# reczoo/RecBox

Hardware: AMD Instinct MI355X
Metric: samples/sec fwd+bwd, Criteo-shaped batch 65 536; embedding HBM GB/s vs roofline (higher is better)
Workload: dtype f32; 1 GPU; FM (recbox.ranking) Criteo-shaped 26 sparse + 13 dense, dim 16, batch 65536 per GPU, uniform ids (8 distinct batches resident in HBM, replayed in rotation), fused path, hipGraph replay (one captured step per resident batch), dense-grad autograd contract (persistent grad buffer, rows of the previous step re-zeroed), no optimiser step; global_batch=65536, batch_per_gpu=65536, parallelism=dp1

## Files before the change

include/recbox_hip.h:

```cpp
#ifndef RECBOX_HIP_H
#define RECBOX_HIP_H

#include <stddef.h>
#include <stdint.h>

#ifdef __cplusplus
extern "C" {
#endif

#define RBX_VERSION 124
#define RBX_MAX_FIELDS 64
#define RBX_NO_ID INT64_MIN

typedef enum {
  RBX_OK = 0,
  RBX_ERR_INVALID = -1,
  RBX_ERR_LAUNCH = -2,
  RBX_ERR_WORKSPACE = -3,
  RBX_ERR_UNSUPPORTED = -4
} rbx_status_t;

typedef enum { RBX_I32 = 0, RBX_I64 = 1, RBX_F32 = 2, RBX_F64 = 3 } rbx_dtype_t;

typedef enum {
  RBX_FIELD_CATEGORICAL = 0,
  RBX_FIELD_NUMERIC = 1,
  RBX_FIELD_DENSE = 2
} rbx_field_kind_t;

typedef enum {
  RBX_POOL_NONE = 0,
  RBX_POOL_SUM = 1,
  RBX_POOL_MEAN_VALUE = 2,
  RBX_POOL_MEAN_ID = 3,
  RBX_POOL_SUM_ID = 4,
  RBX_POOL_CONCAT = 5,
  RBX_POOL_MAX = 6
} rbx_pool_t;

typedef struct rbx_field {
  const void*  ids;
  const float* table;
  float*       grad;
  int64_t      ids_stride_b;
  int64_t      ids_stride_l;
  int64_t      vocab;
  int64_t      padding_idx;
  int64_t      mask_id;
  int64_t      out_off;
  int32_t      dim;
  int32_t      seq_len;
  int32_t      ids_dtype;
  int32_t      kind;
  int32_t      pool;
  float        eps;
  int64_t      table_stride;
} rbx_field_t;

const char* rbx_last_error(void);
int rbx_version(void);

int rbx_embed_fwd(const rbx_field_t* fields, int32_t n_fields, int64_t batch,
                  float* d_out, int64_t out_stride_b, float* d_row_scale,
                  int32_t* d_status, void* stream);

size_t rbx_embed_bwd_workspace_size(const rbx_field_t* fields, int32_t n_fields, int64_t batch);
int rbx_embed_sort(const rbx_field_t* fields, int32_t n_fields, int64_t batch,
                   void* d_workspace, size_t workspace_bytes, int32_t* d_status, void* stream);
int rbx_embed_bwd(const rbx_field_t* fields, int32_t n_fields, int64_t batch,
                  const float* d_dout, int64_t out_stride_b, const float* d_row_scale,
                  int32_t accumulate, void* d_workspace, size_t workspace_bytes, void* stream);
int rbx_embed_bwd_indexed(const rbx_field_t* fields, int32_t n_fields, int64_t batch,
                          const float* d_dout, int64_t out_stride_b, const int32_t* d_dout_index,
                          const float* d_row_scale, int32_t accumulate, void* d_workspace, size_t workspace_bytes,
                          void* stream);

#define RBX_MAX_BAGS 32
typedef struct rbx_bag {
  const void*  indices;
  const void*  offsets;
  const float* table;
  float*       grad;
  int64_t      nnz;
  int64_t      indices_stride;
  int64_t      vocab;
  int64_t      padding_idx;
  int64_t      mask_id;
  int64_t      out_off;
  int32_t      dim;
  int32_t      indices_dtype;
  int32_t      offsets_dtype;
  int32_t      pool;
  float        eps;
  int32_t      reserved;
} rbx_bag_t;
int rbx_embed_csr_fwd(const rbx_bag_t* bags, int32_t n_bags, int64_t batch, float* d_out, int64_t out_stride_b,
                      float* d_row_scale, int32_t* d_status, void* stream);
size_t rbx_embed_csr_bwd_workspace_size(const rbx_bag_t* bags, int32_t n_bags, int64_t batch);
int rbx_embed_csr_sort(const rbx_bag_t* bags, int32_t n_bags, int64_t batch, void* d_workspace, size_t workspace_bytes,
                       int32_t* d_status, void* stream);
int rbx_embed_csr_bwd(const rbx_bag_t* bags, int32_t n_bags, int64_t batch, const float* d_dout, int64_t out_stride_b,
                      const float* d_row_scale, int32_t accumulate, void* d_workspace, size_t workspace_bytes,
                      void* stream);
int rbx_embed_csr_fwd_weighted(const rbx_bag_t* bags, int32_t n_bags, int64_t batch, const float* const* d_weights,
                               float* d_out, int64_t out_stride_b, int32_t* d_status, void* stream);
int rbx_embed_csr_sort_weighted(const rbx_bag_t* bags, int32_t n_bags, int64_t batch, void* d_workspace,
                                size_t workspace_bytes, int32_t* d_status, void* stream);
int rbx_embed_csr_bwd_weighted(const rbx_bag_t* bags, int32_t n_bags, int64_t batch, const float* const* d_weights,
                               const float* d_dout, int64_t out_stride_b, int32_t accumulate, void* d_workspace,
                               size_t workspace_bytes, void* stream);
int rbx_embed_csr_weight_grad(const rbx_bag_t* bags, int32_t n_bags, int64_t batch, const float* d_dout,
                              int64_t out_stride_b, float* const* d_dweights, int32_t* d_status, void* stream);
int rbx_embed_csr_rezero(const rbx_bag_t* bags, int32_t n_bags, int64_t batch, void* d_workspace, size_t workspace_bytes,
                         void* stream);
struct rbx_opt;
int rbx_embed_csr_sparse_update(const rbx_bag_t* bags, int32_t n_bags, int64_t batch, const void* d_workspace,
                                size_t workspace_bytes, const struct rbx_opt* opt, float* const* d_state1,
                                float* const* d_state2, int32_t clear_grad, void* stream);
size_t rbx_embed_csr_fwd_max_workspace_size(const rbx_bag_t* bags, int32_t n_bags, int64_t batch, int64_t long_threshold);
int rbx_embed_csr_fwd_max(const rbx_bag_t* bags, int32_t n_bags, int64_t batch, int64_t long_threshold, float* d_out,
                          int64_t out_stride_b, int32_t* d_argpos, int64_t arg_stride_b, void* d_workspace,
                          size_t workspace_bytes, int32_t* d_status, void* stream);
int rbx_embed_csr_bwd_max(const rbx_bag_t* bags, int32_t n_bags, int64_t batch, const float* d_dout, int64_t out_stride_b,
                          const int32_t* d_argpos, int64_t arg_stride_b, int32_t accumulate, void* d_workspace,
                          size_t workspace_bytes, void* stream);

#define RBX_CSR_SEGMENT 256
#define RBX_CSR_WS_SEGMENTS 0
#define RBX_CSR_WS_LONG_BAGS 1
size_t rbx_embed_csr_fwd_long_workspace_size(const rbx_bag_t* bags, int32_t n_bags, int64_t batch, int64_t long_threshold);
int rbx_embed_csr_fwd_long(const rbx_bag_t* bags, int32_t n_bags, int64_t batch, int64_t long_threshold, float* d_out,
                           int64_t out_stride_b, float* d_row_scale, void* d_workspace, size_t workspace_bytes,
                           int32_t* d_status, void* stream);
int rbx_embed_csr_fwd_weighted_long(const rbx_bag_t* bags, int32_t n_bags, int64_t batch, int64_t long_threshold,
                                    const float* const* d_weights, float* d_out, int64_t out_stride_b, void* d_workspace,
                                    size_t workspace_bytes, int32_t* d_status, void* stream);
int rbx_embed_csr_weight_grad_long(const rbx_bag_t* bags, int32_t n_bags, int64_t batch, int64_t long_threshold,
                                   const float* d_dout, int64_t out_stride_b, float* const* d_dweights, void* d_workspace,
                                   size_t workspace_bytes, int32_t* d_status, void* stream);

int rbx_interaction_fwd(const float* d_emb, int64_t emb_stride_b, int64_t batch, int32_t n_fields, int32_t dim,
                        int32_t mode, float* d_out, void* stream);
int rbx_interaction_bwd(const float* d_emb, int64_t emb_stride_b, const float* d_dout, int64_t batch, int32_t n_fields,
                        int32_t dim, int32_t mode, float* d_demb, int64_t demb_stride_b, void* stream);

int rbx_pairmul_fwd(const float* d_left, const float* d_right, int64_t batch, int32_t n_fields, int32_t dim,
                    int32_t per_pair, float* d_out, void* stream);
int rbx_pairmul_bwd(const float* d_left, const float* d_right, const float* d_dout, int64_t batch, int32_t n_fields,
                    int32_t dim, int32_t per_pair, float* d_dleft, float* d_dright, void* stream);

int rbx_fm_fwd(const rbx_field_t* emb, const rbx_field_t* lr, int32_t n_fields, int64_t batch,
               const float* d_lr_bias, const float* d_extra, int32_t n_extra, int32_t extra_stride,
               int32_t extra_lr_off, const int32_t* d_extra_index, int64_t extra_rows, float* d_logit,
               float* d_prob, float* d_sum, int32_t* d_status, void* stream);
int rbx_fm_extra_bwd(const float* d_dlogit, const float* d_sum, const float* d_extra, int64_t batch,
                     int32_t n_extra, int32_t dim, int32_t extra_stride, int32_t extra_lr_off,
                     const int32_t* d_extra_index, int64_t extra_rows, float* d_dextra, void* stream);

size_t rbx_route_workspace_size(int64_t n_lookups, int32_t world);
int rbx_route(const rbx_field_t* tables, int32_t n_tables, int64_t batch, int32_t world, int64_t capacity,
              const int64_t* d_base, int64_t* d_send, int32_t* d_slot, uint8_t* d_overflow, void* d_workspace,
              size_t workspace_bytes, void* stream);
int rbx_route32(const rbx_field_t* tables, int32_t n_tables, int64_t batch, int32_t world, int64_t capacity,
                const int64_t* d_base, int32_t* d_send, int32_t* d_slot, uint8_t* d_overflow, void* d_workspace,
                size_t workspace_bytes, void* stream);

typedef struct rbx_shard_geom {
  int32_t world;
  int32_t dim;
  int32_t n_rows;
  int32_t n_pool;
  int64_t batch;
  int64_t cap_rows;
  int64_t cap_pool;
} rbx_shard_geom_t;
size_t rbx_shard_int_chunk(const rbx_shard_geom_t* geom);
size_t rbx_shard_float_rows(const rbx_shard_geom_t* geom);
size_t rbx_shard_route_workspace_size(const rbx_shard_geom_t* geom, int32_t pool_seq_len);
int rbx_shard_route(const rbx_shard_geom_t* geom, const rbx_field_t* row_fields, const rbx_field_t* pool_field,
                    const int64_t* d_base, int32_t* d_send, int32_t* d_slot, float* d_inv, uint8_t* d_overflow,
                    int32_t* d_status, void* d_workspace, size_t workspace_bytes, void* stream);
int rbx_shard_serve(const rbx_shard_geom_t* geom, const int32_t* d_recv, const float* d_weight, int64_t n_local_rows,
                    float* d_back, int32_t* d_keys, int32_t* d_src, int32_t* d_status, void* stream);
int rbx_shard_combine_fwd(const rbx_shard_geom_t* geom, const float* d_back, const int32_t* d_slot, const float* d_inv,
                          float* d_out, int64_t out_stride_b, const int64_t* col_off, void* stream);
int rbx_shard_combine_bwd(const rbx_shard_geom_t* geom, const float* d_dout, int64_t dout_stride_b,
                          const int64_t* col_off, const int32_t* d_slot, const float* d_inv, float* d_gsend,
                          void* stream);
size_t rbx_fm_bwd_workspace_size(const rbx_field_t* emb, const rbx_field_t* lr, int32_t n_fields, int64_t batch);
int rbx_fm_sort(const rbx_field_t* emb, const rbx_field_t* lr, int32_t n_fields, int64_t batch,
                void* d_workspace, size_t workspace_bytes, int32_t* d_status, void* stream);
int rbx_fm_sort_phases(const rbx_field_t* emb, const rbx_field_t* lr, int32_t n_fields, int64_t batch,
                       void* d_workspace, size_t workspace_bytes, int32_t* d_status, int32_t phases, void* stream);
int rbx_fm_bwd(const rbx_field_t* emb, const rbx_field_t* lr, int32_t n_fields, int64_t batch,
               const float* d_dlogit, const float* d_sum, float* d_dbias, int32_t accumulate,
               int32_t phases, void* d_workspace, size_t workspace_bytes, void* stream);
int rbx_fm_quad(int32_t enable);
int rbx_sort_chained(int32_t enable);
int rbx_fm_rezero(const rbx_field_t* emb, const rbx_field_t* lr, int32_t n_fields, int64_t batch,
                  void* d_workspace, size_t workspace_bytes, void* stream);
int rbx_fm_head(const rbx_field_t* emb, const rbx_field_t* lr, int32_t n_fields, int64_t batch,
                const void* d_rezero_workspace, size_t rezero_workspace_bytes, void* d_sort_workspace,
                size_t sort_workspace_bytes, int32_t* d_status, void* stream);
int rbx_sort_share(const rbx_field_t* src_a, const rbx_field_t* src_b, int32_t src_n, int32_t src_is_fm,
                   const void* d_src_workspace, const rbx_field_t* dst_a, const rbx_field_t* dst_b, int32_t dst_n,
                   int32_t dst_is_fm, void* d_dst_workspace, size_t dst_workspace_bytes, int64_t batch, void* stream);
int rbx_embed_rezero(const rbx_field_t* fields, int32_t n_fields, int64_t batch, void* d_workspace,
                     size_t workspace_bytes, void* stream);

typedef enum { RBX_OPT_SGD = 0, RBX_OPT_ADAGRAD = 1, RBX_OPT_ADAM = 2 } rbx_opt_kind_t;
typedef struct rbx_opt {
  int32_t kind;
  float   lr;
  float   beta1, beta2;
  float   eps;
  float   weight_decay;
  const float* d_step_size;
} rbx_opt_t;
int rbx_opt_advance(int32_t kind, float lr, float beta1, float beta2, float lr_decay, float* d_t, float* d_step_size,
// ... 327 lines not shown
```

recbox_amd/_lib.py:

```python
import ctypes
import os

HERE = os.path.dirname(os.path.abspath(__file__))
LIB_PATH = os.environ.get("RECBOX_HIP_LIB") or os.path.join(HERE, "lib", "librecbox_hip.so")

RBX_MAX_FIELDS = 64
RBX_NO_ID = -(1 << 63)

RBX_OK, RBX_ERR_INVALID, RBX_ERR_LAUNCH, RBX_ERR_WORKSPACE, RBX_ERR_UNSUPPORTED = 0, -1, -2, -3, -4
RBX_I32, RBX_I64, RBX_F32, RBX_F64 = 0, 1, 2, 3
RBX_MASK_U8 = 4
FIELD_CATEGORICAL, FIELD_NUMERIC, FIELD_DENSE = 0, 1, 2
POOL_NONE, POOL_SUM, POOL_MEAN_VALUE, POOL_MEAN_ID, POOL_SUM_ID, POOL_CONCAT, POOL_MAX = 0, 1, 2, 3, 4, 5, 6
INTERACTION_MODES = {"product_sum": 0, "bi_interaction": 1, "inner_product": 2, "elementwise_product": 3}
FM_SORT_IDS, FM_SORT_TIER_B, FM_SORT_TIER_A = 1, 2, 4
FM_BWD_TABLES, FM_BWD_NUMERIC, FM_BWD_STORE, FM_BWD_SKIP_TIER_A, FM_BWD_SKIP_TIER_B = 1, 2, 4, 8, 16


class rbx_field_t(ctypes.Structure):
    _fields_ = [("ids", ctypes.c_void_p),
                ("table", ctypes.c_void_p),
                ("grad", ctypes.c_void_p),
                ("ids_stride_b", ctypes.c_int64),
                ("ids_stride_l", ctypes.c_int64),
                ("vocab", ctypes.c_int64),
                ("padding_idx", ctypes.c_int64),
                ("mask_id", ctypes.c_int64),
                ("out_off", ctypes.c_int64),
                ("dim", ctypes.c_int32),
                ("seq_len", ctypes.c_int32),
                ("ids_dtype", ctypes.c_int32),
                ("kind", ctypes.c_int32),
                ("pool", ctypes.c_int32),
                ("eps", ctypes.c_float),
                ("table_stride", ctypes.c_int64)]


RBX_MAX_BAGS = 32
STATUS_BAD_ID, STATUS_BAD_OFFSETS = 1, 2
CSR_SEGMENT = 256
CSR_WS_SEGMENTS, CSR_WS_LONG_BAGS = 0, 1


class rbx_bag_t(ctypes.Structure):
    _fields_ = [("indices", ctypes.c_void_p),
                ("offsets", ctypes.c_void_p),
                ("table", ctypes.c_void_p),
                ("grad", ctypes.c_void_p),
                ("nnz", ctypes.c_int64),
                ("indices_stride", ctypes.c_int64),
                ("vocab", ctypes.c_int64),
                ("padding_idx", ctypes.c_int64),
                ("mask_id", ctypes.c_int64),
                ("out_off", ctypes.c_int64),
                ("dim", ctypes.c_int32),
                ("indices_dtype", ctypes.c_int32),
                ("offsets_dtype", ctypes.c_int32),
                ("pool", ctypes.c_int32),
                ("eps", ctypes.c_float),
                ("reserved", ctypes.c_int32)]


class rbx_shard_geom_t(ctypes.Structure):
    _fields_ = [("world", ctypes.c_int32), ("dim", ctypes.c_int32), ("n_rows", ctypes.c_int32),
                ("n_pool", ctypes.c_int32), ("batch", ctypes.c_int64), ("cap_rows", ctypes.c_int64),
                ("cap_pool", ctypes.c_int64)]


class rbx_opt_t(ctypes.Structure):
    _fields_ = [("kind", ctypes.c_int32), ("lr", ctypes.c_float), ("beta1", ctypes.c_float), ("beta2", ctypes.c_float),
                ("eps", ctypes.c_float), ("weight_decay", ctypes.c_float), ("d_step_size", ctypes.c_void_p)]


OPT_SGD, OPT_ADAGRAD, OPT_ADAM = 0, 1, 2


class rbx_rowcopy_t(ctypes.Structure):
    _fields_ = [("src", ctypes.c_void_p), ("dst", ctypes.c_void_p), ("row_bytes", ctypes.c_int64)]


_P = ctypes.c_void_p
_FP = ctypes.POINTER(rbx_field_t)
_BP = ctypes.POINTER(rbx_bag_t)
_RP = ctypes.POINTER(rbx_rowcopy_t)
_GP = ctypes.POINTER(rbx_shard_geom_t)
_OP = ctypes.POINTER(rbx_opt_t)
_PP = ctypes.POINTER(ctypes.c_void_p)
_u64 = ctypes.c_uint64
_i32, _i64, _sz, _f32 = ctypes.c_int32, ctypes.c_int64, ctypes.c_size_t, ctypes.c_float
_IP = ctypes.POINTER(ctypes.c_int32)
_LP = ctypes.POINTER(ctypes.c_int64)

SIGNATURES = {
    "rbx_last_error": (ctypes.c_char_p, []),
    "rbx_version": (ctypes.c_int, []),
    "rbx_embed_fwd": (ctypes.c_int, [_FP, _i32, _i64, _P, _i64, _P, _P, _P]),
    "rbx_embed_bwd_workspace_size": (_sz, [_FP, _i32, _i64]),
    "rbx_embed_sort": (ctypes.c_int, [_FP, _i32, _i64, _P, _sz, _P, _P]),
    "rbx_embed_bwd": (ctypes.c_int, [_FP, _i32, _i64, _P, _i64, _P, _i32, _P, _sz, _P]),
    "rbx_embed_bwd_indexed": (ctypes.c_int, [_FP, _i32, _i64, _P, _i64, _P, _P, _i32, _P, _sz, _P]),
    "rbx_embed_csr_fwd": (ctypes.c_int, [_BP, _i32, _i64, _P, _i64, _P, _P, _P]),
    "rbx_embed_csr_bwd_workspace_size": (_sz, [_BP, _i32, _i64]),
    "rbx_embed_csr_sort": (ctypes.c_int, [_BP, _i32, _i64, _P, _sz, _P, _P]),
    "rbx_embed_csr_bwd": (ctypes.c_int, [_BP, _i32, _i64, _P, _i64, _P, _i32, _P, _sz, _P]),
    "rbx_embed_csr_fwd_weighted": (ctypes.c_int, [_BP, _i32, _i64, _PP, _P, _i64, _P, _P]),
    "rbx_embed_csr_sort_weighted": (ctypes.c_int, [_BP, _i32, _i64, _P, _sz, _P, _P]),
    "rbx_embed_csr_bwd_weighted": (ctypes.c_int, [_BP, _i32, _i64, _PP, _P, _i64, _i32, _P, _sz, _P]),
    "rbx_embed_csr_weight_grad": (ctypes.c_int, [_BP, _i32, _i64, _P, _i64, _PP, _P, _P]),
    "rbx_embed_csr_rezero": (ctypes.c_int, [_BP, _i32, _i64, _P, _sz, _P]),
    "rbx_embed_csr_sparse_update": (ctypes.c_int, [_BP, _i32, _i64, _P, _sz, _OP, _PP, _PP, _i32, _P]),
    "rbx_embed_csr_fwd_long_workspace_size": (_sz, [_BP, _i32, _i64, _i64]),
    "rbx_embed_csr_fwd_long": (ctypes.c_int, [_BP, _i32, _i64, _i64, _P, _i64, _P, _P, _sz, _P, _P]),
    "rbx_embed_csr_fwd_weighted_long": (ctypes.c_int, [_BP, _i32, _i64, _i64, _PP, _P, _i64, _P, _sz, _P, _P]),
    "rbx_embed_csr_weight_grad_long": (ctypes.c_int, [_BP, _i32, _i64, _i64, _P, _i64, _PP, _P, _sz, _P, _P]),
    "rbx_embed_csr_fwd_max_workspace_size": (_sz, [_BP, _i32, _i64, _i64]),
    "rbx_embed_csr_fwd_max": (ctypes.c_int, [_BP, _i32, _i64, _i64, _P, _i64, _P, _i64, _P, _sz, _P, _P]),
    "rbx_embed_csr_bwd_max": (ctypes.c_int, [_BP, _i32, _i64, _P, _i64, _P, _i64, _i32, _P, _sz, _P]),
    "rbx_shard_int_chunk": (_sz, [_GP]),
    "rbx_shard_float_rows": (_sz, [_GP]),
    "rbx_shard_route_workspace_size": (_sz, [_GP, _i32]),
    "rbx_shard_route": (ctypes.c_int, [_GP, _FP, _FP, _P, _P, _P, _P, _P, _P, _P, _sz, _P]),
    "rbx_shard_serve": (ctypes.c_int, [_GP, _P, _P, _i64, _P, _P, _P, _P, _P]),
    "rbx_shard_combine_fwd": (ctypes.c_int, [_GP, _P, _P, _P, _P, _i64, ctypes.POINTER(ctypes.c_int64), _P]),
    "rbx_shard_combine_bwd": (ctypes.c_int, [_GP, _P, _i64, ctypes.POINTER(ctypes.c_int64), _P, _P, _P, _P]),
    "rbx_interaction_fwd": (ctypes.c_int, [_P, _i64, _i64, _i32, _i32, _i32, _P, _P]),
    "rbx_interaction_bwd": (ctypes.c_int, [_P, _i64, _P, _i64, _i32, _i32, _i32, _P, _i64, _P]),
    "rbx_fm_fwd": (ctypes.c_int, [_FP, _FP, _i32, _i64, _P, _P, _i32, _i32, _i32, _P, _i64, _P, _P, _P, _P, _P]),
    "rbx_fm_extra_bwd": (ctypes.c_int, [_P, _P, _P, _i64, _i32, _i32, _i32, _i32, _P, _i64, _P, _P]),
    "rbx_route_workspace_size": (_sz, [_i64, _i32]),
    "rbx_route": (ctypes.c_int, [_FP, _i32, _i64, _i32, _i64, _P, _P, _P, _P, _P, _sz, _P]),
    "rbx_route32": (ctypes.c_int, [_FP, _i32, _i64, _i32, _i64, _P, _P, _P, _P, _P, _sz, _P]),
    "rbx_fm_bwd_workspace_size": (_sz, [_FP, _FP, _i32, _i64]),
    "rbx_fm_sort": (ctypes.c_int, [_FP, _FP, _i32, _i64, _P, _sz, _P, _P]),
    "rbx_fm_sort_phases": (ctypes.c_int, [_FP, _FP, _i32, _i64, _P, _sz, _P, _i32, _P]),
    "rbx_embed_sparse_update": (ctypes.c_int, [_FP, _i32, _i64, _P, _sz, _OP, _PP, _PP, _P]),
    "rbx_opt_advance": (ctypes.c_int, [_i32, _f32, _f32, _f32, _f32, _P, _P, _P]),
    "rbx_fm_sparse_update": (ctypes.c_int, [_FP, _FP, _i32, _i64, _P, _sz, _OP, _PP, _PP, _PP, _PP, _P]),
    "rbx_comm_bind": (ctypes.c_int, [_P, _P, _P, _P, _P]),
    "rbx_all_to_all": (ctypes.c_int, [_P, _P, _P, _sz, _i32, _P]),
    "rbx_comm_bind_collectives": (ctypes.c_int, [_P, _P, _P]),
    "rbx_all_reduce": (ctypes.c_int, [_P, _P, _P, _sz, _i32, _i32, _P]),
    "rbx_all_gather": (ctypes.c_int, [_P, _P, _P, _sz, _P]),
    "rbx_embed_rezero": (ctypes.c_int, [_FP, _i32, _i64, _P, _sz, _P]),
    "rbx_sort_share": (ctypes.c_int, [_FP, _FP, _i32, _i32, _P, _FP, _FP, _i32, _i32, _P, _sz, _i64, _P]),
    "rbx_rowscale": (ctypes.c_int, [_P, _P, _P, _i64, _i32, _f32, _P, _P]),
    "rbx_rowscale_seq": (ctypes.c_int, [_P, _P, _i64, _P, _i64, _i32, _f32, _P, _P]),
    "rbx_seq_colsum_workspace_size": (_sz, [_i64, _i32, _i32]),
    "rbx_seq_colsum": (ctypes.c_int, [_P, _P, _i64, _i32, _i32, _P, _P, _sz, _P]),
    "rbx_sum_prefix": (ctypes.c_int, [_P, _i64, _P, _i64, _P, _i64, _i64, _i32, _i32, _P, _i64, _P]),
    "rbx_fm_quad": (ctypes.c_int, [_i32]),
    "rbx_sort_chained": (ctypes.c_int, [_i32]),
    "rbx_fm_rezero": (ctypes.c_int, [_FP, _FP, _i32, _i64, _P, _sz, _P]),
    "rbx_fm_head": (ctypes.c_int, [_FP, _FP, _i32, _i64, _P, _sz, _P, _sz, _P, _P]),
    "rbx_fm_bwd": (ctypes.c_int, [_FP, _FP, _i32, _i64, _P, _P, _P, _i32, _i32, _P, _sz, _P]),
    "rbx_gatherdot_fwd": (ctypes.c_int, [_FP, _i32, _i64, _P, _i64, _f32, _P, _P, _P]),
    "rbx_gatherdot_bwd_workspace_size": (_sz, [_FP, _i32, _i64]),
    "rbx_gatherdot_sort": (ctypes.c_int, [_FP, _i32, _i64, _P, _sz, _P, _P]),
    "rbx_gatherdot_bwd": (ctypes.c_int, [_FP, _i32, _i64, _P, _i64, _P, _f32, _P, _i64, _i32, _P, _sz, _P]),
    "rbx_negsample": (ctypes.c_int, [_i64, _i64, _i32, _u64, _u64, _P, _P, _P, _P, _P, _P]),
    "rbx_negsample_checked": (ctypes.c_int, [_i64, _i64, _i32, _u64, _u64, _P, _P, _P, _P, _i64, _P, _P, _P]),
    "rbx_gather_rows": (ctypes.c_int, [_RP, _i32, _P, _i64, _i64, _P, _P]),
    "rbx_topk_workspace_size": (_sz, [_i64, _i64, _i32]),
    "rbx_topk": (ctypes.c_int, [_P, _P, _i64, _i64, _i64, _i32, _P, _P, _P, _sz, _P]),
    "rbx_penalize_members": (ctypes.c_int, [_P, _i64, _i32, _P, _P, _P, ctypes.c_double, _P, _P]),
    "rbx_membership": (ctypes.c_int, [_P, _i64, _i32, _P, _P, _P, _P, _P]),
    "rbx_search_ip_workspace_size": (_sz, [_i64, _i64, _i32, _i32]),
    "rbx_search_ip": (ctypes.c_int, [_P, _i64, _i64, _P, _i64, _i32, _i32, _P, _P, _P, _P, _sz, _P]),
    "rbx_batchnorm_workspace_size": (_sz, [_i64, _i32]),
    "rbx_batchnorm_fwd": (ctypes.c_int, [_P, _i64, _i32, _P, _P, _f32, _i32, _f32, _P, _P, _i32, _P, _P, _P, _P, _sz, _P]),
    "rbx_batchnorm_bwd": (ctypes.c_int, [_P, _P, _P, _i64, _i32, _P, _P, _P, _i32, _P, _P, _P, _P, _sz, _P]),
    "rbx_batchnorm_prelu_fwd": (ctypes.c_int, [_P, _i64, _i32, _P, _P, _P, _i32, _f32, _i32, _f32, _P, _P, _P, _P, _P, _P, _sz, _P]),
    "rbx_batchnorm_prelu_bwd": (ctypes.c_int, [_P, _P, _i64, _i32, _P, _P, _P, _i32, _P, _P, _i32, _P, _P, _P, _P, _P, _sz, _P]),
    "rbx_batchnorm_stats": (ctypes.c_int, [_P, _i64, _i32, _P, _P, _sz, _P]),
    "rbx_batchnorm_apply": (ctypes.c_int, [_P, _i64, _i32, _P, _P, _P, _P, _i32, _P, _P]),
    "rbx_batchnorm_bwd_reduce": (ctypes.c_int, [_P, _P, _P, _i64, _i32, _P, _P, _P, _P, _P, _sz, _P]),
    "rbx_batchnorm_bwd_dx": (ctypes.c_int, [_P, _P, _P, _i64, _i32, _P, _P, _P, _P, _P, _i64, _P, _P]),
    "rbx_cin_outer_fwd": (ctypes.c_int, [_P, _P, _i64, _i32, _i32, _i32, _P, _P]),
    "rbx_cin_outer_bwd": (ctypes.c_int, [_P, _P, _P, _i64, _i32, _i32, _i32, _P, _P, _P]),
    "rbx_act_workspace_size": (_sz, [_i64, _i32]),
    "rbx_prelu_fwd": (ctypes.c_int, [_P, _i64, _i32, _P, _i32, _P, _P]),
    "rbx_prelu_bwd": (ctypes.c_int, [_P, _P, _i64, _i32, _P, _i32, _P, _P, _P, _sz, _P]),
    "rbx_dropout": (ctypes.c_int, [_P, _i64, _f32, _u64, _P, _P, _P]),
    "rbx_dice_fwd": (ctypes.c_int, [_P, _i64, _i32, _P, _f32, _i32, _f32, _P, _P, _P, _P, _P, _P, _sz, _P]),
    "rbx_dice_bwd": (ctypes.c_int, [_P, _P, _i64, _i32, _P, _P, _P, _i32, _P, _P, _P, _sz, _P]),
    "rbx_layernorm_fwd": (ctypes.c_int, [_P, _i64, _i32, _P, _P, _f32, _P, _P, _P, _P]),
    "rbx_layernorm_bwd_workspace_size": (_sz, [_i64, _i32]),
    "rbx_layernorm_bwd": (ctypes.c_int, [_P, _P, _i64, _i32, _P, _P, _P, _P, _P, _P, _P, _sz, _P]),
    "rbx_cross_fwd": (ctypes.c_int, [_P, _P, _P, _P, _i64, _i32, _i32, _P, _P]),
    "rbx_cross_bwd": (ctypes.c_int, [_P, _P, _P, _i64, _i32, _i32, _P, _P, _P]),
    "rbx_bce_workspace_size": (_sz, [_i64]),
    "rbx_bce_mean_fwd": (ctypes.c_int, [_P, _P, _i64, _P, _P, _sz, _P]),
    "rbx_bce_mean_bwd": (ctypes.c_int, [_P, _P, _P, _i64, _P, _P]),
    "rbx_sigmoid_bce_mean": (ctypes.c_int, [_P, _P, _i64, _f32, _P, _P, _P, _P, _sz, _P]),
    "rbx_scale_by_scalar": (ctypes.c_int, [_P, _P, _i64, _P, _P]),
    "rbx_sigmoid_bce_mean_onepass": (ctypes.c_int, [_P, _P, _i64, _f32, _P, _P, _P, _P, _sz, _P, _P]),
    "rbx_pairmul_fwd": (ctypes.c_int, [_P, _P, _i64, _i32, _i32, _i32, _P, _P]),
    "rbx_pairmul_bwd": (ctypes.c_int, [_P, _P, _P, _i64, _i32, _i32, _i32, _P, _P, _P]),
    "rbx_l2norm_fwd": (ctypes.c_int, [_P, _i64, _i32, _f32, _P, _P, _P]),
    "rbx_l2norm_fwd_strided": (ctypes.c_int, [_P, _i64, _i64, _i64, _i32, _f32, _P, _P, _P]),
    "rbx_cosdot_fwd": (ctypes.c_int, [_P, _P, _i64, _i64, _i32, _i32, _f32, _f32, _P, _P, _P]),
    "rbx_cosdot_bwd": (ctypes.c_int, [_P, _P, _i64, _P, _P, _i64, _i32, _i32, _f32, _P, _P, _i64, _P]),
    "rbx_l2norm_bwd": (ctypes.c_int, [_P, _P, _P, _i64, _i32, _P, _P]),
    "rbx_pairdot_fwd": (ctypes.c_int, [_P, _P, _i64, _i32, _i32, _f32, _P, _P]),
    "rbx_pairdot_bwd": (ctypes.c_int, [_P, _P, _P, _i64, _i32, _i32, _f32, _P, _P, _P]),
    "rbx_linear_fwd": (ctypes.c_int, [_P, _i64, _P, _P, _i64, _i32, _i32, _i32, _P, _P]),
    "rbx_linear_bwd_workspace_size": (_sz, [_i64, _i32, _i32, _i32]),
    "rbx_linear_fwd_fused": (ctypes.c_int, [_P, _i64, _P, _P, _i64, _i32, _i32, _i32, _P, _i64, _P, _P, _i64, _P]),
    "rbx_linear_dx_fused": (ctypes.c_int, [_P, _i64, _P, _i64, _i32, _i32, _P, _i64, _P, _i64, _P, _i64, _P]),
    "rbx_linear_dx_scaled": (ctypes.c_int, [_P, _i64, _P, _i64, _i32, _i32, _P, _i64, _P, _i64, _P, _P, _i64, _P]),
    "rbx_seqblock_qkv_fwd": (ctypes.c_int, [_P, _i64, _P, _P, ctypes.c_float, _P, _P, _P, _P, _P, _P, _P, _P]),
    "rbx_seqblock_ffn_fwd": (ctypes.c_int, [_P, _P, _P, _P, _P, _i64, _P, _P, ctypes.c_float, _P, _P, _P, _P, _P, _P, _P, _P, _P,
                                            _P, _P, _P, _P, _P, _P]),
    "rbx_seqblock_ffn_bwd_workspace_size": (_sz, [_i64]),
    "rbx_seqblock_ffn_bwd": (ctypes.c_int, [_P, _P, _P, _P, _P, _P, _i64, _P, _P, _P, _P, _P, _P, _P, _P, _P, _P, _P, _P, _sz, _P]),
    "rbx_seqblock_attn_in_bwd_workspace_size": (_sz, [_i64]),
    "rbx_seqblock_attn_in_bwd": (ctypes.c_int, [_P, _P, _P, _P, _P, _P, _i64, _P, _P, _P, _f32, _P, _P, _P, _P, _sz, _P]),
    "rbx_seqblock_attn_out_bwd_workspace_size": (_sz, [_i64]),
    "rbx_seqblock_attn_out_bwd": (ctypes.c_int, [_P, _P, _i64, _P, _P, _P, _P, _P, _sz, _P]),
    "rbx_seqblock_inproj_dw_workspace_size": (_sz, [_i64]),
    "rbx_seqblock_inproj_dw": (ctypes.c_int, [_P, _P, _P, _P, _P, _i64, _P, _P, _P, _P, _P, _sz, _P]),
    "rbx_linear_dwdb_scaled": (ctypes.c_int, [_P, _i64, _P, _i64, _P, _i64, _i32, _i32, _P, _P, _P, _sz, _P]),
    "rbx_fm_sum_fwd": (ctypes.c_int, [_P, _i64, _i64, _i32, _i32, _P, _P, _P]),
    "rbx_fm_sum_lr_fwd": (ctypes.c_int, [_P, _i64, _i64, _i32, _i32, _P, _P, _P, _P, _P, _P]),
    "rbx_linear_dx_deepfm": (ctypes.c_int, [_P, _i64, _P, _i64, _i32, _i32, _P, _i64, _P, _i32, _i32, _P, _P, _P, _P, _i64,
                                            _P]),
    "rbx_linear_bwd": (ctypes.c_int, [_P, _i64, _P, _P, _P, _i64, _i32, _i32, _i32, _P, _i64, _P, _P, _P, _sz, _P]),
    "rbx_split_bf16_size": (_sz, [_i32, _i32, _i32]),
    "rbx_split_bf16": (ctypes.c_int, [_P, _i64, _i32, _i32, _i32, _P, _P]),
    "rbx_split_register": (ctypes.c_int, [_P, _P, _i32, _i32, _i32]),
    "rbx_split_unregister": (ctypes.c_int, [_P]),
    "rbx_gemm_bx6_count": (ctypes.c_uint64, []),
    "rbx_attn_fwd": (ctypes.c_int, [_P, _P, _P, _P, _i64, _i32, _i32, _i32, _f32, _i32, _f32, _P, _P, _P, _P]),
    "rbx_attn_bwd": (ctypes.c_int, [_P, _P, _P, _P, _P, _P, _P, _i64, _i32, _i32, _i32, _f32, _i32, _f32,
                                    _P, _P, _P, _P, _P]),
    "rbx_attn_dropout_fwd": (ctypes.c_int, [_P, _P, _P, _P, _i64, _i32, _i32, _i32, _f32, _i32, _f32, _f32, _u64, _P, _P, _P,
                                            _P, _P]),
    "rbx_attn_dropout_bwd": (ctypes.c_int, [_P, _P, _P, _P, _P, _P, _P, _i64, _i32, _i32, _i32, _f32, _i32, _f32, _f32, _u64,
                                            _P, _P, _P, _P, _P, _P]),
    "rbx_attn_dropout_mask": (ctypes.c_int, [_i64, _i32, _i32, _f32, _u64, _P, _P, _P]),
    "rbx_attn_packed_fwd": (ctypes.c_int, [_P, _i64, _P, _i64, _P, _i64, _i64, _i32, _i32, _i32, _f32, _i32, _f32, _u64, _P,
                                           _P, _i64, _P, _P]),
    "rbx_attn_packed_bwd": (ctypes.c_int, [_P, _i64, _P, _i64, _P, _i64, _P, _i64, _P, _i64, _P, _i64, _i32, _i32, _i32,
                                           _f32, _i32, _f32, _u64, _P, _P, _i64, _P, _i64, _P, _i64, _P, _P]),
    "rbx_loss_workspace_size": (_sz, [_i64]),
    "rbx_softmax_ce_fwd": (ctypes.c_int, [_P, _i64, _i64, _i32, _P, _P, _P, _P, _P, _sz, _P]),
    "rbx_softmax_ce_bwd": (ctypes.c_int, [_P, _i64, _i64, _i32, _P, _P, _P, _P, _P]),
    "rbx_pair_logsigmoid_fwd": (ctypes.c_int, [_P, _P, _P, _i64, _f32, _P, _P, _sz, _P]),
    "rbx_pair_logsigmoid_bwd": (ctypes.c_int, [_P, _P, _P, _P, _i64, _f32, _P, _P, _P]),
    "rbx_pool_fwd": (ctypes.c_int, [_P, _P, _i64, _i32, _i32, _i32, _i32, _f32, _P, _P, _P]),
    "rbx_pool_bwd": (ctypes.c_int, [_P, _P, _P, _i64, _i32, _i32, _i32, _P, _P]),
# ... 67 lines not shown
```

recbox_amd/csrc/rbx_bwd_common.h:

```cpp
#pragma once
#include "rbx_internal.h"

namespace rbx {

constexpr int kSortThreads = 256;
#define RBX_SORT_ITEMS 8
constexpr int kSortItems = RBX_SORT_ITEMS;
constexpr int kSortTile = kSortThreads * kSortItems;
constexpr int kChainTiles = 64;
constexpr int kChainPasses = 4;
constexpr int kRadix = 256;
#define RBX_MAX_RADIX_BITS 8
constexpr int kMaxRadixBits = RBX_MAX_RADIX_BITS;
#define RBX_CHUNK 40
constexpr int kChunk = RBX_CHUNK;
constexpr unsigned kLocalBits = 26;
constexpr unsigned kLocalMask = (1u << kLocalBits) - 1u;
constexpr int kNumSamples = 256;

struct KeyField {
  const void* ids;
  long long stride_b;
  int stride_l;
  int vocab;
  int mask_id;
  int pad_id;
  unsigned row_base;
  unsigned lk_off;
  short seq_len;
  unsigned char dtype, pool;
  int reserved;
};
struct KeyPack { KeyField f[RBX_MAX_FIELDS]; };

struct RedField {
  float* grad;
  float* grad2;
  const float* table;
  unsigned row_base;
  int out_off;
  short dim;
  short seq_len;
  unsigned char pool, slot;
  short reserved;
  int table_stride;
  int reserved2;
};
struct RedPack { RedField f[RBX_MAX_FIELDS]; };

struct SegPack {
  unsigned tile0[RBX_MAX_FIELDS + 1];
  unsigned lk0[RBX_MAX_FIELDS + 1];
  unsigned row0[RBX_MAX_FIELDS];
  unsigned char first_pass[RBX_MAX_FIELDS];
  int n;
};
static_assert(sizeof(KeyPack) + sizeof(SegPack) + 96 <= 4096, "build_keys_kernel's arguments must fit the 4 KiB kernarg segment");

__device__ __forceinline__ void seg_of_tile(const SegPack& S, unsigned tile, int* seg, unsigned* first, unsigned* count) {
  int lo = 0, hi = S.n - 1;
  while (lo < hi) {
    const int mid = (lo + hi + 1) >> 1;
    if (S.tile0[mid] <= tile) lo = mid; else hi = mid - 1;
  }
  *seg = lo;
  const unsigned f = S.lk0[lo] + (tile - S.tile0[lo]) * static_cast<unsigned>(kSortTile);
  const unsigned end = S.lk0[lo + 1];
  *first = f;
  *count = (end - f < static_cast<unsigned>(kSortTile)) ? end - f : static_cast<unsigned>(kSortTile);
}

template <int RB>
__device__ __forceinline__ unsigned seg_digit(unsigned key, unsigned sentinel, unsigned row0, int shift) {
  const unsigned local = (key == sentinel) ? 0xFFFFFFFFu : key - row0;
  return (local >> shift) & ((1u << RB) - 1u);
}

struct NumField {
  const void* ids;
  float* grad;
  long long stride_b;
  int out_off;
  short dim;
  unsigned char dtype, reserved;
};
struct NumPack { NumField f[RBX_MAX_FIELDS]; };

struct BwdPlan {
  int n_cat = 0, n_num = 0;
  KeyPack keys;
  RedPack red;
  NumPack num;
  unsigned n_lookups = 0;
  unsigned total_rows = 0;
  int passes = 0;
  int radix_bits = 8;
  SegPack segs;
  int max_dim = 1;
  bool vec = true;
  size_t off_keys[2], off_vals[2], off_hist, off_ssum, off_head, off_tail, off_flags, off_fin, off_long, off_num, bytes;
  bool chained = false;
  unsigned n_tiles = 0, n_chunks = 0, num_blocks = 0;
  unsigned long_cap = kCUs * 2;
  int chunk = kChunk;
  int sum_stride = 1;
};


int make_plan(const rbx_field_t* fields, int n, int64_t B, const float* dout, int64_t stride_b, BwdPlan* p,
              int extra_dim = 0, const unsigned long long* lookups_of = nullptr);
int run_sort(const BwdPlan& p, char* ws, int* d_status, hipStream_t s);
int run_sort_passes(const BwdPlan& p, char* ws, hipStream_t s);
int generic_reduce(const BwdPlan& p, const float* dout, int64_t stride_b, const int32_t* index, const float* row_scale,
                   int64_t B, int accumulate, char* ws, hipStream_t s);

int csr_bwd_plan(const rbx_bag_t* bags, int n, int64_t batch, BwdPlan* p, size_t* bytes);

template <int G, int NV, bool VEC>
struct Frag {
  static constexpr int W = VEC ? 4 : 1;
  float a[NV * W];
  __device__ __forceinline__ void zero() {
#pragma unroll
    for (int i = 0; i < NV * W; ++i) a[i] = 0.f;
  }
  __device__ __forceinline__ void fma_from(const float* row, int dim, int lane_g, float w) {
#pragma unroll
    for (int u = 0; u < NV; ++u) {
      const int e = (lane_g + u * G) * W;
      if (e < dim) {
        if constexpr (VEC) {
          const float4 t = *reinterpret_cast<const float4*>(row + e);
          a[u * 4 + 0] += w * t.x; a[u * 4 + 1] += w * t.y; a[u * 4 + 2] += w * t.z; a[u * 4 + 3] += w * t.w;
        } else {
          a[u] += w * row[e];
        }
      }
    }
  }
  __device__ __forceinline__ void add_from(const float* row, int dim, int lane_g) { fma_from(row, dim, lane_g, 1.0f); }
  __device__ __forceinline__ void load_from(const float* row, int dim, int lane_g) {
#pragma unroll
    for (int u = 0; u < NV; ++u) {
      int e = (lane_g + u * G) * W;
      e = e < dim ? e : dim - W;
      if constexpr (VEC) {
        const float4 t = *reinterpret_cast<const float4*>(row + e);
        a[u * 4 + 0] = t.x; a[u * 4 + 1] = t.y; a[u * 4 + 2] = t.z; a[u * 4 + 3] = t.w;
      } else {
        a[u] = row[e];
      }
    }
  }
  __device__ __forceinline__ void load_from_nt(const float* row, int dim, int lane_g) {
    typedef float v4f __attribute__((ext_vector_type(4)));
#pragma unroll
    for (int u = 0; u < NV; ++u) {
      int e = (lane_g + u * G) * W;
      e = e < dim ? e : dim - W;
      if constexpr (VEC) {
        const v4f t = __builtin_nontemporal_load(reinterpret_cast<const v4f*>(row + e));
        a[u * 4 + 0] = t.x; a[u * 4 + 1] = t.y; a[u * 4 + 2] = t.z; a[u * 4 + 3] = t.w;
      } else {
        a[u] = __builtin_nontemporal_load(row + e);
      }
    }
  }
  __device__ __forceinline__ void scale(float w) {
#pragma unroll
    for (int i = 0; i < NV * W; ++i) a[i] *= w;
  }
  __device__ __forceinline__ void add_from_nt(const float* row, int dim, int lane_g) {
    typedef float v4f __attribute__((ext_vector_type(4)));
#pragma unroll
    for (int u = 0; u < NV; ++u) {
      const int e = (lane_g + u * G) * W;
      if (e < dim) {
        if constexpr (VEC) {
          const v4f t = __builtin_nontemporal_load(reinterpret_cast<const v4f*>(row + e));
          a[u * 4 + 0] += t.x; a[u * 4 + 1] += t.y; a[u * 4 + 2] += t.z; a[u * 4 + 3] += t.w;
        } else {
          a[u] += __builtin_nontemporal_load(row + e);
        }
      }
    }
  }
  __device__ __forceinline__ void store_nt(float* row, int dim, int lane_g) const {
    typedef float v4f __attribute__((ext_vector_type(4)));
#pragma unroll
    for (int u = 0; u < NV; ++u) {
      const int e = (lane_g + u * G) * W;
      if (e < dim) {
        if constexpr (VEC) {
          v4f t;
          t.x = a[u * 4]; t.y = a[u * 4 + 1]; t.z = a[u * 4 + 2]; t.w = a[u * 4 + 3];
          __builtin_nontemporal_store(t, reinterpret_cast<v4f*>(row + e));
        } else {
          __builtin_nontemporal_store(a[u], row + e);
        }
      }
    }
  }
  __device__ __forceinline__ void store(float* row, int dim, int lane_g) const {
#pragma unroll
    for (int u = 0; u < NV; ++u) {
      const int e = (lane_g + u * G) * W;
      if (e < dim) {
        if constexpr (VEC) {
          *reinterpret_cast<float4*>(row + e) = make_float4(a[u * 4], a[u * 4 + 1], a[u * 4 + 2], a[u * 4 + 3]);
        } else {
          row[e] = a[u];
        }
      }
    }
  }
  __device__ __forceinline__ void accumulate_into(float* row, int dim, int lane_g) const {
#pragma unroll
    for (int u = 0; u < NV; ++u) {
      const int e = (lane_g + u * G) * W;
      if (e < dim) {
        if constexpr (VEC) {
          float4 t = *reinterpret_cast<float4*>(row + e);
          t.x += a[u * 4]; t.y += a[u * 4 + 1]; t.z += a[u * 4 + 2]; t.w += a[u * 4 + 3];
          *reinterpret_cast<float4*>(row + e) = t;
        } else {
          row[e] += a[u];
        }
      }
    }
  }
};

constexpr int kFlagFin = 1;
constexpr int kFlagPass = 2;
constexpr int kFlagZero = 4;


}
```

recbox_amd/csrc/rbx_embed_bwd.hip:

```cpp
#include <stdlib.h>
#include "rbx_segreduce.h"

namespace rbx {

static size_t align_up(size_t v, size_t a) { return (v + a - 1) / a * a; }

static int g_sort_chained = -1;
static bool sort_chained_on() {
  if (g_sort_chained < 0) {
    const char* e = getenv("RBX_SORT_CHAINED");
    g_sort_chained = (e != nullptr && e[0] == '0') ? 0 : 1;
  }
  return g_sort_chained != 0;
}

int make_plan(const rbx_field_t* fields, int n, int64_t B, const float* dout, int64_t stride_b, BwdPlan* p,
              int extra_dim, const unsigned long long* lookups_of) {
  if (fields == nullptr || n <= 0 || n > RBX_MAX_FIELDS) return fail(RBX_ERR_INVALID, "bad field array");
  FieldPack tmp;
  int rc = pack_fields(fields, n, B, true, &tmp);
  if (rc != RBX_OK) return rc;
  unsigned long long lookups = 0, rows = 0;
  const float* seen_table[RBX_MAX_FIELDS];
  unsigned seen_base[RBX_MAX_FIELDS];
  int seen_dim[RBX_MAX_FIELDS];
  long long seen_vocab[RBX_MAX_FIELDS];
  int n_seen = 0;
  int field_table[RBX_MAX_FIELDS];
  unsigned field_lookups[RBX_MAX_FIELDS];
  p->vec = (stride_b % 4 == 0) && ((reinterpret_cast<uintptr_t>(dout) & 15) == 0);
  for (int i = 0; i < n; ++i) {
    const rbx_field_t& f = fields[i];
    if (f.kind == RBX_FIELD_DENSE || f.grad == nullptr) continue;
    if (f.dim > p->max_dim) p->max_dim = f.dim;
    if (f.dim % 4 != 0 || f.out_off % 4 != 0 || (reinterpret_cast<uintptr_t>(f.grad) & 15) != 0) p->vec = false;
    if (f.kind == RBX_FIELD_NUMERIC) {
      NumField& nf = p->num.f[p->n_num++];
      nf.ids = f.ids;
      nf.grad = f.grad;
      nf.stride_b = f.ids_stride_b;
      nf.out_off = static_cast<int>(f.out_off);
      nf.dim = static_cast<short>(f.dim);
      nf.dtype = static_cast<unsigned char>(f.ids_dtype);
      continue;
    }
    const unsigned long long n_lk = lookups_of != nullptr ? lookups_of[i] : static_cast<unsigned long long>(B) * f.seq_len;
    if (n_lk > kLocalMask) return fail(RBX_ERR_UNSUPPORTED, "field %d: B*seq_len=%llu exceeds 2^26 per call", i, n_lk);
    int hit = -1;
    for (int s = 0; s < n_seen; ++s)
      if (seen_table[s] == f.table) hit = s;
    if (hit >= 0 && (seen_dim[hit] != f.dim || seen_vocab[hit] != f.vocab))
      return fail(RBX_ERR_INVALID, "field %d shares a table with different vocab/dim", i);
    if (hit < 0) {
      hit = n_seen++;
      seen_table[hit] = f.table;
      seen_base[hit] = static_cast<unsigned>(rows);
      seen_dim[hit] = f.dim;
      seen_vocab[hit] = f.vocab;
      rows += static_cast<unsigned long long>(f.vocab);
    }
    const int c = p->n_cat++;
    field_table[c] = hit;
    field_lookups[c] = static_cast<unsigned>(n_lk);
    KeyField& kf = p->keys.f[c];
    kf.ids = f.ids;
    kf.stride_b = f.ids_stride_b;
    kf.stride_l = static_cast<int>(f.ids_stride_l);
    kf.vocab = static_cast<int>(f.vocab);
    kf.mask_id = tmp.f[i].mask_id;
    kf.pad_id = tmp.f[i].pad_id;
    kf.row_base = seen_base[hit];
    kf.lk_off = static_cast<unsigned>(lookups);
    kf.seq_len = static_cast<short>(f.seq_len);
    kf.dtype = static_cast<unsigned char>(f.ids_dtype);
    kf.pool = static_cast<unsigned char>(f.pool);
    kf.reserved = 0;
    RedField& rf = p->red.f[c];
    rf.grad = f.grad;
    rf.grad2 = nullptr;
    rf.table = f.table;
    rf.row_base = seen_base[hit];
    rf.out_off = static_cast<int>(f.out_off);
    rf.dim = static_cast<short>(f.dim);
    rf.seq_len = static_cast<short>(f.seq_len);
    rf.pool = static_cast<unsigned char>(f.pool);
    rf.slot = static_cast<unsigned char>(i);
    rf.reserved = 0;
    rf.table_stride = f.dim;
    rf.reserved2 = 0;
    lookups += n_lk;
  }
  if (lookups >= (1ull << 31) || rows >= (1ull << 31))
    return fail(RBX_ERR_UNSUPPORTED, "too many lookups/rows for one call (%llu / %llu)", lookups, rows);
  if (p->n_cat > 0 && pow2_ceil(p->vec ? p->max_dim / 4 : p->max_dim) > 256)
    return fail(RBX_ERR_UNSUPPORTED, "embedding dim %d too large for one lane group (%s units)", p->max_dim,
                p->vec ? "float4" : "scalar");
  p->n_lookups = static_cast<unsigned>(lookups);
  p->total_rows = static_cast<unsigned>(rows);
  {
    int last_field_of_table[RBX_MAX_FIELDS];
    for (int c = 0; c < p->n_cat; ++c) last_field_of_table[field_table[c]] = c;
    SegPack& S = p->segs;
    S.n = 0;
    unsigned tiles = 0, lk = 0;
    unsigned long long max_rows = 1;
    unsigned long long rows_of_seg[RBX_MAX_FIELDS];
    int c = 0;
    while (c < p->n_cat) {
      int end = last_field_of_table[field_table[c]];
      unsigned long long seg_rows = 0;
      unsigned seg_lk = 0;
      const unsigned row0 = p->keys.f[c].row_base;
      int t_lo = field_table[c], t_hi = field_table[c];
      for (int k = c; k <= end; ++k) {
        if (last_field_of_table[field_table[k]] > end) end = last_field_of_table[field_table[k]];
        if (field_table[k] > t_hi) t_hi = field_table[k];
        if (field_table[k] < t_lo) t_lo = field_table[k];
        seg_lk += field_lookups[k];
      }
      for (int t = t_lo; t <= t_hi; ++t) seg_rows += static_cast<unsigned long long>(seen_vocab[t]);
      if (seg_lk > 0) {
        S.tile0[S.n] = tiles;
        S.lk0[S.n] = lk;
        S.row0[S.n] = row0;
        rows_of_seg[S.n] = seg_rows;
        ++S.n;
        tiles += (seg_lk + kSortTile - 1) / kSortTile;
        lk += seg_lk;
        if (seg_rows > max_rows) max_rows = seg_rows;
      }
      c = end + 1;
    }
    S.tile0[S.n] = tiles;
    S.lk0[S.n] = lk;
    p->n_tiles = tiles;
    unsigned max_nt = 0;
    for (int g = 0; g < S.n; ++g)
      if (S.tile0[g + 1] - S.tile0[g] > max_nt) max_nt = S.tile0[g + 1] - S.tile0[g];
    p->chained = max_nt <= static_cast<unsigned>(kChainTiles);
    int bits = 1;
    while ((1ull << bits) <= max_rows) ++bits;
    p->passes = (bits + kMaxRadixBits - 1) / kMaxRadixBits;
    const int per = (bits + p->passes - 1) / p->passes;
    p->radix_bits = per <= 8 ? 8 : (per <= 10 ? 10 : 11);
    for (int g = 0; g < S.n; ++g) {
      int sb = 1;
      while ((1ull << sb) <= rows_of_seg[g]) ++sb;
      const int need = (sb + p->radix_bits - 1) / p->radix_bits;
      S.first_pass[g] = static_cast<unsigned char>(p->passes - need);
    }
  }
  {
    int c = static_cast<int>(p->n_lookups / 32768u) / 8 * 8;
    if (c < 16) c = 16;
    if (c > kChunk) c = kChunk;
    p->chunk = c;
  }
  p->n_chunks = (p->n_lookups + p->chunk - 1) / p->chunk;
  p->num_blocks = static_cast<unsigned>((B + kNumSamples - 1) / kNumSamples);
  size_t o = 0;
  const size_t nl = align_up(static_cast<size_t>(p->n_lookups) * 4, 256);
  p->off_keys[0] = o; o += nl;
  p->off_keys[1] = o; o += nl;
  p->off_vals[0] = o; o += nl;
  p->off_vals[1] = o; o += nl;
  const size_t radix = static_cast<size_t>(1) << p->radix_bits;
  p->chained = sort_chained_on() && p->chained && p->passes <= kChainPasses && p->radix_bits == 8;
  p->off_hist = o;
  o += p->chained ? align_up((2 * static_cast<size_t>(p->n_tiles) * radix + p->n_tiles + static_cast<size_t>(p->segs.n) * radix) *
                             p->passes * 4, 256)
                  : align_up(static_cast<size_t>(p->n_tiles) * radix * 4 + 4, 256);
  p->off_ssum = o; o += align_up((static_cast<size_t>(p->n_tiles) * radix / 4096 + 2) * 4, 256);
  p->sum_stride = p->max_dim + extra_dim;
  p->off_head = o; o += align_up(static_cast<size_t>(p->n_chunks) * p->sum_stride * 4, 256);
  p->off_tail = o; o += align_up(static_cast<size_t>(p->n_chunks) * p->sum_stride * 4, 256);
  p->off_flags = o; o += align_up(static_cast<size_t>(p->n_chunks) * 4, 256);
  p->off_fin = o; o += align_up((2 * static_cast<size_t>(p->n_chunks) + 3 + kLongSlots) * 4, 256);
  p->off_long = o; o += align_up(static_cast<size_t>(kLongSlots) * p->sum_stride * 4, 256);
  p->off_num = o; o += align_up(static_cast<size_t>(p->n_num) * p->num_blocks * p->max_dim * 4, 256);
  p->bytes = o + 256;
  return RBX_OK;
}


template <int RB>
__global__ __launch_bounds__(kSortThreads) void build_keys_kernel(const KeyPack P, const int n_cat, const SegPack S,
                                                         const unsigned sentinel, unsigned* __restrict__ keys0,
                                                         unsigned* __restrict__ vals0, unsigned* __restrict__ keys1,
                                                         unsigned* __restrict__ vals1, int* __restrict__ status,
                                                         unsigned* __restrict__ fin, unsigned* __restrict__ hist,
                                                         const int chain_passes, const unsigned n_tiles) {
  constexpr int R = 1 << RB;
  constexpr int kCP = (RB == 8) ? kChainPasses : 1;
  if (blockIdx.x == 0 && threadIdx.x == 0) {
    fin[0] = 0;
    fin[1] = 0;
    fin[2] = 0;
  }
  __shared__ KeyField sf[RBX_MAX_FIELDS];
  {
    const int words = n_cat * static_cast<int>(sizeof(KeyField) / 4);
    const int* src = reinterpret_cast<const int*>(&P);
    int* dst = reinterpret_cast<int*>(sf);
    for (int i = threadIdx.x; i < words; i += blockDim.x) dst[i] = src[i];
  }
  __shared__ unsigned cnt[kCP][R];
  for (int d = threadIdx.x; d < kCP * R; d += kSortThreads) (&cnt[0][0])[d] = 0;
  __syncthreads();
  int seg;
  unsigned tile0, tile_n;
  seg_of_tile(S, blockIdx.x, &seg, &tile0, &tile_n);
  const unsigned row0 = S.row0[seg];
  const int fp = S.first_pass[seg];
  unsigned* __restrict__ keys = (fp & 1) ? keys1 : keys0;
  unsigned* __restrict__ vals = (fp & 1) ? vals1 : vals0;
#pragma unroll
  for (int it = 0; it < kSortItems; ++it) {
    const unsigned off = it * kSortThreads + threadIdx.x;
    if (off >= tile_n) break;
    const unsigned j = tile0 + off;
    int lo = 0, hi = n_cat - 1;
    while (lo < hi) {
      const int mid = (lo + hi + 1) >> 1;
      if (sf[mid].lk_off <= j) lo = mid; else hi = mid - 1;
    }
    const KeyField& fd = sf[lo];
    const unsigned local = j - fd.lk_off;
    const unsigned L = static_cast<unsigned>(fd.seq_len);
    const unsigned b = local / L;
    const unsigned l = local - b * L;
    const long long id = load_id(fd.ids, static_cast<long long>(b) * fd.stride_b + static_cast<long long>(l) * fd.stride_l,
                                 fd.dtype);
    unsigned key = sentinel;
    if (id < 0 || id >= fd.vocab) {
      if (status != nullptr) atomicOr(status, 1);
    } else {
      const bool id_pool = fd.pool == RBX_POOL_MEAN_ID || fd.pool == RBX_POOL_SUM_ID;
      if (id != fd.pad_id && !(id_pool && id == fd.mask_id)) key = fd.row_base + static_cast<unsigned>(id);
    }
    keys[j] = key;
    vals[j] = (static_cast<unsigned>(lo) << kLocalBits) | local;
    if (chain_passes > 0) {
#pragma unroll
      for (int k = 0; k < kCP; ++k)
        if (fp + k < chain_passes) atomicAdd(&cnt[k][seg_digit<RB>(key, sentinel, row0, k * RB)], 1u);
    } else if (fp == 0) {
      atomicAdd(&cnt[0][seg_digit<RB>(key, sentinel, row0, 0)], 1u);
    }
  }
  if (chain_passes > 0) {
    __syncthreads();
    const size_t plane = static_cast<size_t>(n_tiles) * R;
    unsigned* flags = hist + 2 * plane * chain_passes;
    for (int k = 0; fp + k < chain_passes; ++k) {
      unsigned* h = hist + plane * (fp + k) + static_cast<size_t>(blockIdx.x) * R;
      for (int d = threadIdx.x; d < R; d += kSortThreads) h[d] = cnt[k < kCP ? k : 0][d];
      if (threadIdx.x == 0) flags[static_cast<size_t>(fp + k) * n_tiles + blockIdx.x] = 0u;
    }
    return;
  }
  if (fp != 0) return;
  __syncthreads();
  const unsigned t_in = blockIdx.x - S.tile0[seg], nt = S.tile0[seg + 1] - S.tile0[seg];
  unsigned* h = hist + static_cast<size_t>(S.tile0[seg]) * R + t_in;
  for (int d = threadIdx.x; d < R; d += kSortThreads) h[static_cast<size_t>(d) * nt] = cnt[0][d];
}

template <int RB>
__global__ __launch_bounds__(kSortThreads) void radix_hist_kernel(const unsigned* __restrict__ keys, const SegPack S,
                                                                  const unsigned sentinel, const int pass,
                                                                  unsigned* __restrict__ hist) {
  constexpr int R = 1 << RB;
  __shared__ unsigned cnt[R];
  int seg;
  unsigned tile0, tile_n;
  seg_of_tile(S, blockIdx.x, &seg, &tile0, &tile_n);
  if (pass < S.first_pass[seg]) return;
  const int shift = (pass - S.first_pass[seg]) * RB;
  for (int d = threadIdx.x; d < R; d += kSortThreads) cnt[d] = 0;
  __syncthreads();
  const unsigned row0 = S.row0[seg];
#pragma unroll
  for (int i = 0; i < kSortItems; ++i) {
    const unsigned off = i * kSortThreads + threadIdx.x;
    if (off < tile_n) atomicAdd(&cnt[seg_digit<RB>(keys[tile0 + off], sentinel, row0, shift)], 1u);
  }
  __syncthreads();
  const unsigned t_in = blockIdx.x - S.tile0[seg], nt = S.tile0[seg + 1] - S.tile0[seg];
  unsigned* h = hist + static_cast<size_t>(S.tile0[seg]) * R + t_in;
  for (int d = threadIdx.x; d < R; d += kSortThreads) h[static_cast<size_t>(d) * nt] = cnt[d];
}

constexpr int kScanSlice = 4096;
constexpr int kMaxFusedSlices = 4 * kSortThreads;

__device__ __forceinline__ unsigned block_scan_1024x4(unsigned (&v)[4], unsigned* wave_tot, unsigned* total) {
  const int lane = threadIdx.x & 63, wid = threadIdx.x >> 6;
  const unsigned mine = v[0] + v[1] + v[2] + v[3];
  unsigned inc = mine;
#pragma unroll
  for (int o = 1; o < 64; o <<= 1) {
    const unsigned t = __shfl_up(inc, o, 64);
    if (lane >= o) inc += t;
  }
  if (lane == 63) wave_tot[wid] = inc;
  __syncthreads();
  unsigned wbase = 0, all = 0;
#pragma unroll
  for (int w = 0; w < 16; ++w) {
    const unsigned t = wave_tot[w];
    if (w < wid) wbase += t;
    all += t;
  }
  *total = all;
  return wbase + inc - mine;
}

__global__ __launch_bounds__(1024) void radix_scan_local_kernel(unsigned* __restrict__ hist, const unsigned len,
                                                                unsigned* __restrict__ slice_sum) {
  __shared__ unsigned wave_tot[16];
  const unsigned i0 = blockIdx.x * kScanSlice + threadIdx.x * 4;
  unsigned v[4];
#pragma unroll
  for (int k = 0; k < 4; ++k) v[k] = (i0 + k < len) ? hist[i0 + k] : 0u;
  unsigned total;
  unsigned run = block_scan_1024x4(v, wave_tot, &total);
#pragma unroll
  for (int k = 0; k < 4; ++k) {
    if (i0 + k < len) hist[i0 + k] = run;
    run += v[k];
// ... 237 lines not shown
#pragma unroll 8
          for (unsigned t = 0; t < t_in; ++t)
            b += __hip_atomic_load(Ls + static_cast<size_t>(t) * R + threadIdx.x * DPT + q, __ATOMIC_RELAXED,
                                   __HIP_MEMORY_SCOPE_AGENT);
          chain_before[q] = b;
        }
      }
#pragma unroll
      for (int q = 0; q < DPT; ++q) gbase[threadIdx.x * DPT + q] = seg_lk0 + chain_excl[q] + chain_before[q];
    }
  }
  __syncthreads();
#pragma unroll
  for (int s = 0; s < kSteps; ++s) {
    const unsigned off = wid * kPerWave + s * 64 + lane;
    if (off < tile_n) {
      const unsigned d = seg_digit<RB>(k[s], sentinel, row0, shift);
      const unsigned pos = dstart[d] + wcnt[wid][d] + rank[s];
      skey[pos] = k[s];
      sval[pos] = v[s];
    }
  }
  __syncthreads();
#pragma unroll
  for (int i = 0; i < kSortItems; ++i) {
    const unsigned pos = i * kSortThreads + threadIdx.x;
    if (pos < tile_n) {
      const unsigned key = skey[pos];
      const unsigned d = seg_digit<RB>(key, sentinel, row0, shift);
      const unsigned g = gbase[d] + (pos - dstart[d]);
      keys_out[g] = key;
      vals_out[g] = sval[pos];
    }
  }
}

struct GenericPolicy {
  static constexpr bool kHasCount = false;
  struct Args {
    const float* dout;
    long long stride_b;
    const float* row_scale;
    long long B;
    int accumulate;
    const int* index;
  };
  template <class F>
  static __device__ __forceinline__ void contribute(const Args& a, const RedField& fd, unsigned local, int lane_g,
                                                    F& frag, float& cnt) {
    const unsigned L = static_cast<unsigned>(fd.seq_len);
    const unsigned b = local / L;
    const unsigned l = local - b * L;
    const long long brow = (a.index != nullptr) ? static_cast<long long>(a.index[b]) : static_cast<long long>(b);
    const float* src = a.dout + brow * a.stride_b + fd.out_off +
                       (fd.pool == RBX_POOL_CONCAT ? static_cast<long long>(l) * fd.dim : 0ll);
    float w = 1.0f;
    if (fd.pool == RBX_POOL_MEAN_VALUE || fd.pool == RBX_POOL_MEAN_ID)
      w = a.row_scale[static_cast<long long>(fd.slot) * a.B + b];
    frag.fma_from(src, fd.dim, lane_g, w);
    (void)cnt;
  }
  template <class F>
  static __device__ __forceinline__ void prefetch(const Args& a, const RedField& fd, unsigned row, int lane_g, F& pre) {
    if (a.accumulate) pre.add_from(fd.grad + static_cast<size_t>(row) * fd.dim, fd.dim, lane_g);
  }
  template <class F>
  static __device__ __forceinline__ void fetch(const Args& a, const RedField& fd, unsigned local, int lane_g, F& frag, float& w) {
    const unsigned L = static_cast<unsigned>(fd.seq_len);
    const unsigned b = local / L;
    const unsigned l = local - b * L;
    const long long brow = (a.index != nullptr) ? static_cast<long long>(a.index[b]) : static_cast<long long>(b);
    const float* src = a.dout + brow * a.stride_b + fd.out_off +
                       (fd.pool == RBX_POOL_CONCAT ? static_cast<long long>(l) * fd.dim : 0ll);
    w = 1.0f;
    if (fd.pool == RBX_POOL_MEAN_VALUE || fd.pool == RBX_POOL_MEAN_ID)
      w = a.row_scale[static_cast<long long>(fd.slot) * a.B + b];
    frag.load_from(src, fd.dim, lane_g);
  }
  static __device__ __forceinline__ float weight(const Args&, float w) { return w; }
  template <class F>
  static __device__ __forceinline__ void prefetch_raw(const Args& a, const RedField& fd, unsigned row, int lane_g, F& pre) {
    if (a.accumulate) pre.load_from(fd.grad + static_cast<size_t>(row) * fd.dim, fd.dim, lane_g);
  }
  template <class F>
  static __device__ __forceinline__ void flush(const Args&, const RedField& fd, unsigned row, const F& acc, float,
                                               const F& pre, int lane_g) {
    F out = acc;
    frag_add(out, pre);
    out.store_nt(fd.grad + static_cast<size_t>(row) * fd.dim, fd.dim, lane_g);
  }
};

__global__ __launch_bounds__(256) void numeric_partial_kernel(const NumPack P, const long long B,
                                                              const float* __restrict__ dout, const long long stride_b,
                                                              float* __restrict__ partial, const int max_dim,
                                                              const unsigned num_blocks) {
  const NumField fd = P.f[blockIdx.y];
  const int dim = fd.dim;
  __shared__ float red[256];
  const long long b0 = static_cast<long long>(blockIdx.x) * kNumSamples;
  const long long b1 = (b0 + kNumSamples < B) ? b0 + kNumSamples : B;
  for (int dbase = 0; dbase < dim; dbase += 16) {
    const int d = dbase + (threadIdx.x & 15);
    float acc = 0.f;
    if (d < dim) {
      long long b = b0 + (threadIdx.x >> 4);
      for (; b + 48 < b1; b += 64) {
        float xv[4], gv[4];
#pragma unroll
        for (int u = 0; u < 4; ++u) {
          xv[u] = load_value(fd.ids, (b + 16 * u) * fd.stride_b, fd.dtype);
          gv[u] = dout[(b + 16 * u) * stride_b + fd.out_off + d];
        }
#pragma unroll
        for (int u = 0; u < 4; ++u) acc += xv[u] * gv[u];
      }
      for (; b < b1; b += 16) {
        const float x = load_value(fd.ids, b * fd.stride_b, fd.dtype);
        acc += x * dout[b * stride_b + fd.out_off + d];
      }
    }
    red[threadIdx.x] = acc;
    __syncthreads();
    if (threadIdx.x < 16) {
      float t = 0.f;
#pragma unroll
      for (int r = 0; r < 16; ++r) t += red[r * 16 + threadIdx.x];
      if (d < dim) partial[(static_cast<size_t>(blockIdx.y) * num_blocks + blockIdx.x) * max_dim + d] = t;
    }
    __syncthreads();
  }
}

__global__ __launch_bounds__(64) void numeric_final_kernel(const NumPack P, const float* __restrict__ partial,
                                                           const int max_dim, const unsigned num_blocks) {
  const NumField fd = P.f[blockIdx.x];
  const int d = blockIdx.y;
  if (d >= fd.dim) return;
  float t = 0.f;
  for (unsigned k = threadIdx.x; k < num_blocks; k += 64)
    t += partial[(static_cast<size_t>(blockIdx.x) * num_blocks + k) * max_dim + d];
  t = group_sum<64>(t);
  if (threadIdx.x == 0) fd.grad[d] += t;
}

}

extern "C" int rbx_sort_chained(int32_t enable) {
  const int was = rbx::sort_chained_on() ? 1 : 0;
  if (enable >= 0) rbx::g_sort_chained = enable ? 1 : 0;
  return was;
}

extern "C" size_t rbx_embed_bwd_workspace_size(const rbx_field_t* fields, int32_t n_fields, int64_t batch) {
  rbx::BwdPlan p;
  if (rbx::make_plan(fields, n_fields, batch, nullptr, 0, &p) != RBX_OK) return 0;
  return p.bytes;
}

namespace rbx {
template <int RB>
static int run_passes_rb(const BwdPlan& p, char* ws, hipStream_t s) {
  constexpr int R = 1 << RB;
  unsigned* keys[2] = {reinterpret_cast<unsigned*>(ws + p.off_keys[0]), reinterpret_cast<unsigned*>(ws + p.off_keys[1])};
  unsigned* vals[2] = {reinterpret_cast<unsigned*>(ws + p.off_vals[0]), reinterpret_cast<unsigned*>(ws + p.off_vals[1])};
  unsigned* hist = reinterpret_cast<unsigned*>(ws + p.off_hist);
  unsigned* ssum = reinterpret_cast<unsigned*>(ws + p.off_ssum);
  const bool chained = p.chained && RB == 8;
  int rc = RBX_OK;
  int cur = 0;
  for (int pass = 0; pass < p.passes; ++pass) {
    if (chained) {
      hipLaunchKernelGGL((radix_scatter_kernel<RB, true>), dim3(p.n_tiles), dim3(kSortThreads), 0, s, keys[cur], vals[cur],
                         keys[cur ^ 1], vals[cur ^ 1], p.segs, p.total_rows, pass, static_cast<const unsigned*>(nullptr),
                         static_cast<const unsigned*>(nullptr), 0u, false, hist, p.passes, p.n_tiles);
      rc = check_launch("radix pass (chained)");
      if (rc != RBX_OK) return rc;
      cur ^= 1;
      continue;
    }
    if (pass > 0)
      hipLaunchKernelGGL(radix_hist_kernel<RB>, dim3(p.n_tiles), dim3(kSortThreads), 0, s, keys[cur], p.segs, p.total_rows,
                         pass, hist);
    const unsigned hist_len = p.n_tiles * R;
    const unsigned n_slices = (hist_len + kScanSlice - 1) / kScanSlice;
    hipLaunchKernelGGL(radix_scan_local_kernel, dim3(n_slices), dim3(1024), 0, s, hist, hist_len, ssum);
    const bool raw_sums = n_slices <= static_cast<unsigned>(kMaxFusedSlices);
    if (!raw_sums) hipLaunchKernelGGL(radix_scan_sums_kernel, dim3(1), dim3(1024), 0, s, ssum, n_slices);
    hipLaunchKernelGGL((radix_scatter_kernel<RB, false>), dim3(p.n_tiles), dim3(kSortThreads), 0, s, keys[cur], vals[cur],
                       keys[cur ^ 1], vals[cur ^ 1], p.segs, p.total_rows, pass, hist, ssum, n_slices, raw_sums,
                       static_cast<unsigned*>(nullptr), p.passes, p.n_tiles);
    rc = check_launch("radix pass");
    if (rc != RBX_OK) return rc;
    cur ^= 1;
  }
  return RBX_OK;
}

int run_sort_passes(const BwdPlan& p, char* ws, hipStream_t s) {
  switch (p.radix_bits) {
    case 8: return run_passes_rb<8>(p, ws, s);
    case 10: return run_passes_rb<10>(p, ws, s);
    default: return run_passes_rb<11>(p, ws, s);
  }
}

template <int RB>
static int run_sort_rb(const BwdPlan& p, char* ws, int* d_status, hipStream_t s) {
  unsigned* keys[2] = {reinterpret_cast<unsigned*>(ws + p.off_keys[0]), reinterpret_cast<unsigned*>(ws + p.off_keys[1])};
  unsigned* vals[2] = {reinterpret_cast<unsigned*>(ws + p.off_vals[0]), reinterpret_cast<unsigned*>(ws + p.off_vals[1])};
  const bool chained = p.chained && RB == 8;
  hipLaunchKernelGGL(build_keys_kernel<RB>, dim3(p.n_tiles), dim3(kSortThreads), 0, s, p.keys, p.n_cat, p.segs, p.total_rows,
                     keys[0], vals[0], keys[1], vals[1], d_status, reinterpret_cast<unsigned*>(ws + p.off_fin),
                     reinterpret_cast<unsigned*>(ws + p.off_hist), chained ? p.passes : 0, p.n_tiles);
  const int rc = check_launch("build_keys_kernel");
  if (rc != RBX_OK) return rc;
  return run_passes_rb<RB>(p, ws, s);
}

int run_sort(const BwdPlan& p, char* ws, int* d_status, hipStream_t s) {
  if (p.n_lookups == 0) return RBX_OK;
  switch (p.radix_bits) {
    case 8: return run_sort_rb<8>(p, ws, d_status, s);
    case 10: return run_sort_rb<10>(p, ws, d_status, s);
    default: return run_sort_rb<11>(p, ws, d_status, s);
  }
}

int generic_reduce(const BwdPlan& p, const float* dout, int64_t stride_b, const int32_t* index, const float* row_scale,
                   int64_t B, int accumulate, char* ws, hipStream_t s) {
  for (int i = 0; i < p.n_cat; ++i) {
    const unsigned char pool = p.red.f[i].pool;
    if ((pool == RBX_POOL_MEAN_VALUE || pool == RBX_POOL_MEAN_ID) && row_scale == nullptr)
      return fail(RBX_ERR_INVALID, "mean pooling backward needs d_row_scale from the forward");
  }
  const int cur = p.passes & 1;
  const unsigned* keys = reinterpret_cast<const unsigned*>(ws + p.off_keys[cur]);
  const unsigned* vals = reinterpret_cast<const unsigned*>(ws + p.off_vals[cur]);
  const GenericPolicy::Args args = {dout, static_cast<long long>(stride_b), row_scale, static_cast<long long>(B), accumulate,
                                    index};
  return p.vec ? dispatch_reduce<GenericPolicy, true>(p, args, keys, vals, ws, s)
               : dispatch_reduce<GenericPolicy, false>(p, args, keys, vals, ws, s);
}
}

extern "C" int rbx_embed_sort(const rbx_field_t* fields, int32_t n_fields, int64_t batch, void* d_workspace,
                              size_t workspace_bytes, int32_t* d_status, void* stream) {
  using namespace rbx;
  BwdPlan p;
  int rc = make_plan(fields, n_fields, batch, nullptr, 0, &p);
  if (rc != RBX_OK) return rc;
  if (p.n_lookups == 0) return RBX_OK;
  if (d_workspace == nullptr || workspace_bytes < p.bytes)
    return fail(RBX_ERR_WORKSPACE, "workspace %zu B < required %zu B", workspace_bytes, p.bytes);
  return run_sort(p, static_cast<char*>(d_workspace), d_status, as_stream(stream));
}

extern "C" int rbx_embed_rezero(const rbx_field_t* fields, int32_t n_fields, int64_t batch, void* d_workspace,
                                size_t workspace_bytes, void* stream) {
  using namespace rbx;
  if (batch == 0) return RBX_OK;
  BwdPlan p;
  int rc = make_plan(fields, n_fields, batch, nullptr, 0, &p);
  if (rc != RBX_OK) return rc;
  if (p.n_lookups == 0) return RBX_OK;
  if (d_workspace == nullptr || workspace_bytes < p.bytes) return fail(RBX_ERR_WORKSPACE, "embed_rezero: workspace too small");
  return launch_rezero(p, static_cast<const char*>(d_workspace), as_stream(stream));
}

extern "C" int rbx_embed_bwd(const rbx_field_t* fields, int32_t n_fields, int64_t batch, const float* d_dout,
                             int64_t out_stride_b, const float* d_row_scale, int32_t accumulate, void* d_workspace,
                             size_t workspace_bytes, void* stream) {
  return rbx_embed_bwd_indexed(fields, n_fields, batch, d_dout, out_stride_b, nullptr, d_row_scale, accumulate, d_workspace,
                               workspace_bytes, stream);
}

extern "C" int rbx_embed_bwd_indexed(const rbx_field_t* fields, int32_t n_fields, int64_t batch, const float* d_dout,
                                     int64_t out_stride_b, const int32_t* d_dout_index, const float* d_row_scale,
                                     int32_t accumulate, void* d_workspace, size_t workspace_bytes, void* stream) {
  using namespace rbx;
  if (d_dout == nullptr) return fail(RBX_ERR_INVALID, "d_dout is NULL");
  if (batch == 0) return RBX_OK;
  BwdPlan p;
  int rc = make_plan(fields, n_fields, batch, d_dout, out_stride_b, &p);
  if (rc != RBX_OK) return rc;
  if (d_workspace == nullptr || workspace_bytes < p.bytes)
    return fail(RBX_ERR_WORKSPACE, "workspace %zu B < required %zu B", workspace_bytes, p.bytes);
  char* ws = static_cast<char*>(d_workspace);
  hipStream_t s = as_stream(stream);
  if (p.n_lookups > 0) {
    rc = generic_reduce(p, d_dout, out_stride_b, d_dout_index, d_row_scale, batch, accumulate, ws, s);
    if (rc != RBX_OK) return rc;
  }
  if (p.n_num > 0 && d_dout_index != nullptr) return fail(RBX_ERR_UNSUPPORTED, "embed_bwd_indexed: numeric features are not indexed");
  if (p.n_num > 0) {
    float* partial = reinterpret_cast<float*>(ws + p.off_num);
    hipLaunchKernelGGL(numeric_partial_kernel, dim3(p.num_blocks, p.n_num), dim3(256), 0, s, p.num,
                       static_cast<long long>(batch), d_dout, static_cast<long long>(out_stride_b), partial, p.max_dim,
                       p.num_blocks);
    hipLaunchKernelGGL(numeric_final_kernel, dim3(p.n_num, p.max_dim), dim3(64), 0, s, p.num, partial, p.max_dim,
                       p.num_blocks);
    rc = check_launch("numeric grad kernels");
    if (rc != RBX_OK) return rc;
  }
  return RBX_OK;
}
// ... 1 lines not shown
```

recbox_amd/csrc/rbx_embed_csr.hip:

```cpp
#include "rbx_bwd_common.h"
#include "rbx_rowfrag.h"
#include "rbx_segreduce.h"

namespace rbx {

constexpr int kStatusBadId = 1;
constexpr int kStatusBadOffsets = 2;

struct BagK {
  const void* indices;
  const void* offsets;
  const float* table;
  long long idx_stride;
  int nnz;
  int vocab;
  int mask_id;
  int pad_id;
  int out_off;
  short dim;
  unsigned char idx_dtype, off_dtype, pool, slot;
  short reserved;
  float eps;
};
static_assert(sizeof(BagK) == 64, "BagK must stay 64 bytes");
// ... 674 lines not shown
  __syncthreads();
  const unsigned t_in = blockIdx.x - S.tile0[seg], nt = S.tile0[seg + 1] - S.tile0[seg];
  unsigned* h = hist + static_cast<size_t>(S.tile0[seg]) * R + t_in;
  for (int d = threadIdx.x; d < R; d += kSortThreads) h[static_cast<size_t>(d) * nt] = cnt[0][d];
}

struct CsrPlan {
  BwdPlan p;
  BagPack bags;
  BagLookups lk;
  size_t off_map = 0, bytes = 0;
};

static int csr_plan(const rbx_bag_t* bags, int n, int64_t batch, const float* dout, int64_t stride_b, CsrPlan* c) {
  BagK all[RBX_MAX_BAGS];
  int rc = pack_bags(bags, n, batch, all);
  if (rc != RBX_OK) return rc;
  rbx_field_t fields[RBX_MAX_BAGS];
  unsigned long long lookups_of[RBX_MAX_BAGS];
  for (int i = 0; i < n; ++i) {
    const rbx_bag_t& g = bags[i];
    rbx_field_t& f = fields[i];
    f.ids = g.indices != nullptr ? g.indices : static_cast<const void*>(g.table);
    f.table = g.table;
    f.grad = g.grad;
    f.ids_stride_b = g.indices_stride;
    f.ids_stride_l = 0;
    f.vocab = g.vocab;
    f.padding_idx = g.padding_idx;
    f.mask_id = g.mask_id;
    f.out_off = g.out_off;
    f.dim = g.dim;
    f.seq_len = 1;
    f.ids_dtype = g.indices_dtype;
    f.kind = RBX_FIELD_CATEGORICAL;
    f.pool = g.pool == RBX_POOL_MAX ? RBX_POOL_SUM_ID : g.pool;
    f.eps = g.eps;
    f.table_stride = 0;
    lookups_of[i] = static_cast<unsigned long long>(g.nnz);
  }
  rc = make_plan(fields, n, batch, dout, stride_b, &c->p, 0, lookups_of);
  if (rc != RBX_OK) return rc;
  int k = 0;
  for (int i = 0; i < n; ++i) {
    if (bags[i].grad == nullptr) continue;
    c->bags.f[k] = all[i];
    c->lk.lk_off[k] = c->p.keys.f[k].lk_off;
    ++k;
  }
  c->off_map = c->p.bytes;
  c->bytes = c->p.bytes + (static_cast<size_t>(c->p.n_lookups) * 4 + 255) / 256 * 256;
  return RBX_OK;
}

int csr_bwd_plan(const rbx_bag_t* bags, int n, int64_t batch, BwdPlan* p, size_t* bytes) {
  CsrPlan c;
  const int rc = csr_plan(bags, n, batch, nullptr, 0, &c);
  if (rc != RBX_OK) return rc;
  *p = c.p;
  *bytes = c.bytes;
  return RBX_OK;
}

template <int RB, bool POS = false>
static int launch_csr_keys(const CsrPlan& c, char* ws, int* status, hipStream_t s) {
  const BwdPlan& p = c.p;
  const bool chained = p.chained && RB == 8;
  hipLaunchKernelGGL((csr_keys_kernel<RB, POS>), dim3(p.n_tiles), dim3(kSortThreads), 0, s, p.keys, p.n_cat, p.segs, p.total_rows,
                     reinterpret_cast<const int*>(ws + c.off_map), reinterpret_cast<unsigned*>(ws + p.off_keys[0]),
                     reinterpret_cast<unsigned*>(ws + p.off_vals[0]), reinterpret_cast<unsigned*>(ws + p.off_keys[1]),
                     reinterpret_cast<unsigned*>(ws + p.off_vals[1]), status, reinterpret_cast<unsigned*>(ws + p.off_fin),
                     reinterpret_cast<unsigned*>(ws + p.off_hist), chained ? p.passes : 0, p.n_tiles);
  return check_launch("csr_keys_kernel");
}

struct BagPolicyBase {
  static constexpr bool kHasCount = false;
  template <class A>
  static __device__ __forceinline__ float weight(const A&, float w) { return w; }
  template <class A, class F>
  static __device__ __forceinline__ void prefetch(const A& a, const RedField& fd, unsigned row, int lane_g, F& pre) {
    if (a.accumulate) pre.add_from(fd.grad + static_cast<size_t>(row) * fd.dim, fd.dim, lane_g);
  }
  template <class A, class F>
  static __device__ __forceinline__ void prefetch_raw(const A& a, const RedField& fd, unsigned row, int lane_g, F& pre) {
    if (a.accumulate) pre.load_from(fd.grad + static_cast<size_t>(row) * fd.dim, fd.dim, lane_g);
  }
  template <class A, class F>
  static __device__ __forceinline__ void flush(const A&, const RedField& fd, unsigned row, const F& acc, float, const F& pre,
                                               int lane_g) {
    F out = acc;
    frag_add(out, pre);
    out.store_nt(fd.grad + static_cast<size_t>(row) * fd.dim, fd.dim, lane_g);
  }
};

struct WeightedBagPolicy : BagPolicyBase {
  struct Args {
    const float* dout;
    long long stride_b;
    const int* map;
    int accumulate;
    unsigned lk_off[RBX_MAX_BAGS];
    const float* w[RBX_MAX_BAGS];
  };
  template <class F>
  static __device__ __forceinline__ void fetch(const Args& a, const RedField& fd, unsigned pos, int lane_g, F& frag, float& w) {
    const int bag = a.map[a.lk_off[fd.slot] + pos];
    const float* wp = a.w[fd.slot];
    w = (wp != nullptr) ? wp[pos] : 1.0f;
    frag.load_from(a.dout + static_cast<long long>(bag) * a.stride_b + fd.out_off, fd.dim, lane_g);
  }
};

struct MaxBagPolicy : BagPolicyBase {
  struct Args {
    const float* dout;
    long long stride_b;
    const int* argpos;
    long long arg_stride;
    const int* map;
    int accumulate;
    unsigned lk_off[RBX_MAX_BAGS];
  };
  template <int G, int NV, bool VEC>
  static __device__ __forceinline__ void fetch(const Args& a, const RedField& fd, unsigned pos, int lane_g, Frag<G, NV, VEC>& frag,
                                               float& w) {
    const int bag = a.map[a.lk_off[fd.slot] + pos];
    w = 1.0f;
    frag.load_from(a.dout + static_cast<long long>(bag) * a.stride_b + fd.out_off, fd.dim, lane_g);
    const int* __restrict__ arg = a.argpos + static_cast<long long>(bag) * a.arg_stride + fd.out_off;
    const int me = static_cast<int>(pos);
    constexpr int W = VEC ? 4 : 1;
#pragma unroll
    for (int u = 0; u < NV; ++u) {
      int e = (lane_g + u * G) * W;
      e = e < fd.dim ? e : fd.dim - W;
      if constexpr (VEC) {
        const int4 t = *reinterpret_cast<const int4*>(arg + e);
        frag.a[u * 4 + 0] = t.x == me ? frag.a[u * 4 + 0] : 0.f;
        frag.a[u * 4 + 1] = t.y == me ? frag.a[u * 4 + 1] : 0.f;
        frag.a[u * 4 + 2] = t.z == me ? frag.a[u * 4 + 2] : 0.f;
        frag.a[u * 4 + 3] = t.w == me ? frag.a[u * 4 + 3] : 0.f;
      } else {
        frag.a[u] = arg[e] == me ? frag.a[u] : 0.f;
      }
    }
  }
};
template <>
struct ReduceWideBatch<MaxBagPolicy> {
  static constexpr int of(int per_lane) { return per_lane > 8 ? 2 : 4; }
};
template <>
struct ReduceLaneZeros<MaxBagPolicy> {
  static constexpr bool value = true;
};

static int csr_sort(const rbx_bag_t* bags, int n_bags, int64_t batch, void* d_workspace, size_t workspace_bytes,
                    int* d_status, hipStream_t s, bool pos) {
  CsrPlan c;
  int rc = csr_plan(bags, n_bags, batch, nullptr, 0, &c);
  if (rc != RBX_OK) return rc;
  const BwdPlan& p = c.p;
  if (p.n_lookups == 0 || batch == 0) return RBX_OK;
  if (d_workspace == nullptr || workspace_bytes < c.bytes)
    return fail(RBX_ERR_WORKSPACE, "workspace %zu B < required %zu B", workspace_bytes, c.bytes);
  char* ws = static_cast<char*>(d_workspace);
  int* map = reinterpret_cast<int*>(ws + c.off_map);
  if (hipMemsetAsync(map, 0xFF, static_cast<size_t>(p.n_lookups) * 4, s) != hipSuccess)
    return fail(RBX_ERR_LAUNCH, "clearing the lookup -> bag map failed");
  long long bx = (batch + 15) / 16;
  if (bx > kCUs * 8) bx = kCUs * 8;
  hipLaunchKernelGGL(csr_bag_map_kernel, dim3(static_cast<unsigned>(bx), p.n_cat), dim3(256), 0, s, c.bags, c.lk,
                     static_cast<long long>(batch), map, d_status);
  rc = check_launch("csr_bag_map_kernel");
  if (rc != RBX_OK) return rc;
  switch (p.radix_bits) {
    case 8: rc = pos ? launch_csr_keys<8, true>(c, ws, d_status, s) : launch_csr_keys<8>(c, ws, d_status, s); break;
    case 10: rc = pos ? launch_csr_keys<10, true>(c, ws, d_status, s) : launch_csr_keys<10>(c, ws, d_status, s); break;
    default: rc = pos ? launch_csr_keys<11, true>(c, ws, d_status, s) : launch_csr_keys<11>(c, ws, d_status, s); break;
  }
  if (rc != RBX_OK) return rc;
  return run_sort_passes(p, ws, s);
}

static int check_no_trained_mean(const rbx_bag_t* bags, int n, const char* who) {
  for (int i = 0; bags != nullptr && i < n; ++i)
    if (bags[i].grad != nullptr && (bags[i].pool == RBX_POOL_MEAN_ID || bags[i].pool == RBX_POOL_MEAN_VALUE))
      return fail(RBX_ERR_UNSUPPORTED, "%s: bag %d is a mean pool with a gradient; its backward goes through rbx_embed_csr_sort / "
                  "rbx_embed_csr_bwd (d_row_scale)", who, i);
  return RBX_OK;
}

__global__ __launch_bounds__(256) void csr_long_finish_kernel(const BagPack P, const int F, const long long B,
                                                              float* __restrict__ out, const long long stride_b,
                                                              float* __restrict__ row_scale, const LongArgs LA) {
  int n_long;
  long long n_segs;
  long_counts(LA, &n_long, &n_segs);
  const int lane = threadIdx.x & 63;
  for (long long r = static_cast<long long>(blockIdx.x) * 4 + threadIdx.x / 64; r < n_long;
       r += static_cast<long long>(gridDim.x) * 4) {
    const LongRec rec = LA.recs[r];
    if (rec.end <= rec.begin || static_cast<unsigned>(rec.desc) >= static_cast<unsigned>(F)) continue;
    const long long nseg = (static_cast<long long>(rec.end) - rec.begin + kSeg - 1) / kSeg;
    if (rec.seg0 < 0 || rec.seg0 + nseg > n_segs || rec.bag < 0 || rec.bag >= B) continue;
    const BagK& fd = P.f[rec.desc];
    const bool mean = fd.pool == RBX_POOL_MEAN_VALUE || fd.pool == RBX_POOL_MEAN_ID;
    float inv = 1.0f;
    if (mean) {
      float count = 0.f;
      for (long long j = 0; j < nseg; ++j) count += LA.pcnt[rec.seg0 + j];
      inv = 1.0f / (count + fd.eps);
      if (row_scale != nullptr && lane == 0) row_scale[static_cast<long long>(fd.slot) * B + rec.bag] = inv;
    }
    float* dst = out + rec.bag * stride_b + fd.out_off;
    const float* src = LA.part + static_cast<long long>(rec.seg0) * LA.pstride;
    for (int d = lane; d < fd.dim; d += 64) {
      float a = 0.f;
      for (long long j = 0; j < nseg; ++j) a += src[j * LA.pstride + d];
      dst[d] = mean ? a * inv : a;
    }
  }
}

__global__ __launch_bounds__(256) void csr_long_max_finish_kernel(const BagPack P, const int F, const long long B,
                                                                  float* __restrict__ out, const long long stride_b,
                                                                  int* __restrict__ argpos, const long long arg_stride,
                                                                  const int* __restrict__ parg, const LongArgs LA) {
  int n_long;
  long long n_segs;
  long_counts(LA, &n_long, &n_segs);
  const int lane = threadIdx.x & 63;
  for (long long r = static_cast<long long>(blockIdx.x) * 4 + threadIdx.x / 64; r < n_long;
       r += static_cast<long long>(gridDim.x) * 4) {
    const LongRec rec = LA.recs[r];
    if (rec.end <= rec.begin || static_cast<unsigned>(rec.desc) >= static_cast<unsigned>(F)) continue;
    const long long nseg = (static_cast<long long>(rec.end) - rec.begin + kSeg - 1) / kSeg;
    if (rec.seg0 < 0 || rec.seg0 + nseg > n_segs || rec.bag < 0 || rec.bag >= B) continue;
    const BagK& fd = P.f[rec.desc];
    float* dst = out + rec.bag * stride_b + fd.out_off;
    int* adst = argpos + rec.bag * arg_stride + fd.out_off;
    const float* src = LA.part + static_cast<long long>(rec.seg0) * LA.pstride;
    const int* asrc = parg + static_cast<long long>(rec.seg0) * LA.pstride;
    for (int d = lane; d < fd.dim; d += 64) {
      float best = 0.f;
      int at = -1;
      for (long long j = 0; j < nseg; ++j) {
        const int p = asrc[j * LA.pstride + d];
        const float v = src[j * LA.pstride + d];
        if (p >= 0 && (at < 0 || v > best)) {
          best = v;
          at = p;
        }
      }
      dst[d] = best;
      adst[d] = at;
    }
  }
}

struct LongPlan {
  int T = 0, cap_bags = 0, cap_segs = 0, pstride = 4;
  size_t off_recs = 0, off_part = 0, off_cnt = 0, bytes = 0;
};
constexpr size_t kLongHeader = 256;

static int long_plan(const rbx_bag_t* bags, int n, int64_t batch, int64_t threshold, LongPlan* lp) {
  int rc = check_sizes(bags, n, batch, -1);
  if (rc != RBX_OK) return rc;
  if (threshold < 0) return fail(RBX_ERR_INVALID, "negative long_threshold");
  long long cap_bags = 0, cap_segs = 0;
  int dim = 1;
  for (int i = 0; i < n; ++i) {
    const rbx_bag_t& g = bags[i];
    rc = check_sizes(bags, n, batch, i);
    if (rc != RBX_OK) return rc;
    if (g.dim > dim) dim = g.dim;
    if (threshold == 0) continue;
    const long long most = g.nnz / threshold < batch ? g.nnz / threshold : batch;
    cap_bags += most;
    cap_segs += g.nnz / kSeg + most;
  }
  if (cap_bags == 0) cap_segs = 0;
  lp->T = threshold > INT_MAX ? INT_MAX : static_cast<int>(threshold);
  lp->cap_bags = static_cast<int>(cap_bags);
  lp->cap_segs = static_cast<int>(cap_segs);
  lp->pstride = (dim + 3) / 4 * 4;
  auto up = [](size_t v) { return (v + 255) / 256 * 256; };
  lp->off_recs = kLongHeader;
  lp->off_part = lp->off_recs + up(static_cast<size_t>(cap_bags) * sizeof(LongRec));
  lp->off_cnt = lp->off_part + up(static_cast<size_t>(cap_segs) * lp->pstride * 4);
  lp->bytes = lp->off_cnt + up(static_cast<size_t>(cap_segs) * 4);
  return RBX_OK;
}

static LongArgs long_args(const LongPlan& lp, void* ws) {
  char* base = static_cast<char*>(ws);
  LongArgs la;
  la.hdr = reinterpret_cast<unsigned long long*>(base);
  la.recs = reinterpret_cast<LongRec*>(base + lp.off_recs);
  la.part = reinterpret_cast<float*>(base + lp.off_part);
  la.pcnt = reinterpret_cast<float*>(base + lp.off_cnt);
  la.T = lp.T;
  la.cap_bags = lp.cap_bags;
  la.cap_segs = lp.cap_segs;
  la.pstride = lp.pstride;
  la.cls = 0;
  return la;
// ... 362 lines not shown
```

recbox_amd/csrc/rbx_ffm.hip:

```cpp
#include "rbx_segreduce.h"

namespace rbx {

struct FfmField {
  const void* ids;
  const float* table;
  long long stride_b;
  int nblocks;
  int dtype;
};
struct FfmPack { FfmField f[RBX_MAX_FIELDS]; };

constexpr int kFfmMaxPairs = RBX_MAX_FIELDS * (RBX_MAX_FIELDS - 1) / 2;

template <int D4C, bool REDUCE>
__global__ __launch_bounds__(256) void ffm_fwd_kernel(const FfmPack P, const int F, const int D, const long long B,
                                                      float* __restrict__ out, const long long out_stride_b,
                                                      int* __restrict__ status, const int spw, const unsigned n_tasks) {
  typedef float v4f __attribute__((ext_vector_type(4)));
  __shared__ FfmField sf[RBX_MAX_FIELDS];
  __shared__ unsigned short s_pair[kFfmMaxPairs];
  {
    const int words = F * static_cast<int>(sizeof(FfmField) / 4);
    const int* src = reinterpret_cast<const int*>(&P);
    int* dst = reinterpret_cast<int*>(sf);
    for (int i = threadIdx.x; i < words; i += blockDim.x) dst[i] = src[i];
  }
  const int npairs = F * (F - 1) / 2;
  for (int p = threadIdx.x; p < npairs; p += blockDim.x) {
    int i = 0, rem = p;
    while (rem >= F - 1 - i) {
      rem -= F - 1 - i;
      ++i;
    }
    s_pair[p] = static_cast<unsigned short>((i << 8) | (i + 1 + rem));
  }
  __syncthreads();
  const int D4 = D4C > 0 ? D4C : D / 4;
  const int lane = threadIdx.x & 63, wid = threadIdx.x >> 6;
  const unsigned n_waves = gridDim.x * (blockDim.x >> 6);
  for (unsigned task = blockIdx.x * (blockDim.x >> 6) + wid; task < n_tasks; task += n_waves) {
    const long long s0 = static_cast<long long>(task) * spw;
    int x = -1;
    {
      const int sl = lane / F, f = lane - sl * F;
      const long long s = s0 + sl;
      if (sl < spw && s < B) {
        const FfmField& fd = sf[f];
        const long long id = load_id(fd.ids, s * fd.stride_b, fd.dtype);
        if (id >= 0 && id < fd.nblocks) x = static_cast<int>(id);
        else if (status != nullptr) atomicOr(status, 1);
      }
    }
    const int ns = (B - s0 < spw) ? static_cast<int>(B - s0) : spw;
    for (int sl = 0; sl < ns; ++sl) {
      float* __restrict__ orow = out + (s0 + sl) * out_stride_b;
      const int base = sl * F;
      const int units = REDUCE ? npairs : npairs * D4;
      for (int r0 = 0; r0 < units; r0 += 64) {
        const int r = r0 + lane;
        const bool live = r < units;
        const int rr = live ? r : 0;
        const int p = REDUCE ? rr : rr / D4;
        const int d4 = REDUCE ? 0 : rr - p * D4;
        const unsigned ij = s_pair[p];
        const int i = static_cast<int>(ij >> 8), j = static_cast<int>(ij & 255u);
        const int xi = __shfl(x, base + i, 64), xj = __shfl(x, base + j, 64);
        const bool ok = xi >= 0 && xj >= 0;
        const float* ra = sf[i].table + (static_cast<size_t>(xi < 0 ? 0 : xi) * F + j) * D + d4 * 4;
        const float* rb = sf[j].table + (static_cast<size_t>(xj < 0 ? 0 : xj) * F + i) * D + d4 * 4;
        if constexpr (REDUCE) {
          float acc = 0.f;
          for (int q = 0; q < D4; ++q) {
            const float4 a = *reinterpret_cast<const float4*>(ra + q * 4);
            const float4 b = *reinterpret_cast<const float4*>(rb + q * 4);
            acc += a.x * b.x;
            acc += a.y * b.y;
            acc += a.z * b.z;
            acc += a.w * b.w;
          }
          if (live) __builtin_nontemporal_store(ok ? acc : 0.f, orow + r);
        } else {
          const float4 a = *reinterpret_cast<const float4*>(ra);
          const float4 b = *reinterpret_cast<const float4*>(rb);
          v4f o;
          o.x = ok ? a.x * b.x : 0.f;
          o.y = ok ? a.y * b.y : 0.f;
          o.z = ok ? a.z * b.z : 0.f;
          o.w = ok ? a.w * b.w : 0.f;
          if (live) __builtin_nontemporal_store(o, reinterpret_cast<v4f*>(orow + static_cast<size_t>(r) * 4));
        }
      }
    }
  }
}

struct FfmPolicy {
  static constexpr bool kHasCount = false;
  struct Args {
    const FfmField* pack;
    const float* dout;
    long long stride_b;
    int F, D;
    int reduce_sum;
    int accumulate;
  };
  template <int G, int NV>
  static __device__ __forceinline__ void fetch(const Args& a, const RedField& fd, unsigned b, int lane_g,
                                               Frag<G, NV, true>& frag, float& w) {
    w = 1.0f;
    const int i = fd.slot;
    const int F = a.F, D = a.D;
    const int dim = F * D;
    const float* drow = a.dout + static_cast<long long>(b) * a.stride_b;
#pragma unroll
    for (int u = 0; u < NV; ++u) {
      const int e = (lane_g + u * G) * 4;
      const bool in = e < dim;
      const int ec = in ? e : 0;
      const int j0 = ec / D, d = ec - j0 * D;
      const bool off_diag = in && j0 != i;
      const int j = (j0 != i) ? j0 : (i == 0 ? 1 : 0);
      const int lo = i < j ? i : j, hi = i < j ? j : i;
      const int p = lo * F - lo * (lo + 1) / 2 + (hi - lo - 1);
      const FfmField fj = a.pack[j];
      const long long id = load_id(fj.ids, static_cast<long long>(b) * fj.stride_b, fj.dtype);
      const bool ok = off_diag && id >= 0 && id < fj.nblocks;
      const float* row = fj.table + (static_cast<size_t>(ok ? id : 0) * F + i) * D + d;
      const float4 t = *reinterpret_cast<const float4*>(row);
      float4 g;
      if (a.reduce_sum) {
        const float s = drow[p];
        g = make_float4(s, s, s, s);
      } else {
        g = *reinterpret_cast<const float4*>(drow + static_cast<size_t>(p) * D + d);
      }
      frag.a[u * 4 + 0] = ok ? g.x * t.x : 0.f;
      frag.a[u * 4 + 1] = ok ? g.y * t.y : 0.f;
      frag.a[u * 4 + 2] = ok ? g.z * t.z : 0.f;
      frag.a[u * 4 + 3] = ok ? g.w * t.w : 0.f;
    }
  }
  static __device__ __forceinline__ float weight(const Args&, float w) { return w; }
  template <class Fr>
  static __device__ __forceinline__ void prefetch(const Args& a, const RedField& fd, unsigned row, int lane_g, Fr& pre) {
    if (a.accumulate) pre.add_from(fd.grad + static_cast<size_t>(row) * fd.dim, fd.dim, lane_g);
  }
  template <class Fr>
  static __device__ __forceinline__ void prefetch_raw(const Args& a, const RedField& fd, unsigned row, int lane_g, Fr& pre) {
    if (a.accumulate) pre.load_from(fd.grad + static_cast<size_t>(row) * fd.dim, fd.dim, lane_g);
  }
  template <class Fr>
  static __device__ __forceinline__ void flush(const Args&, const RedField& fd, unsigned row, const Fr& acc, float,
                                               const Fr& pre, int lane_g) {
    Fr o = acc;
    frag_add(o, pre);
    o.store_nt(fd.grad + static_cast<size_t>(row) * fd.dim, fd.dim, lane_g);
  }
};
template <>
struct ReduceWideBatch<FfmPolicy> {
  static constexpr int of(int per_lane) { return per_lane >= 16 ? 2 : 4; }
};
template <>
struct ReduceLaneZeros<FfmPolicy> {
  static constexpr bool value = true;
};

__global__ __launch_bounds__(64) void ffm_pack_kernel(const FfmPack P, const int F, FfmField* __restrict__ dst) {
  const int words = F * static_cast<int>(sizeof(FfmField) / 4);
  const int* src = reinterpret_cast<const int*>(&P);
  int* d = reinterpret_cast<int*>(dst);
  for (int i = threadIdx.x; i < words; i += blockDim.x) d[i] = src[i];
}

static size_t ffm_align(size_t v) { return (v + 255) / 256 * 256; }

static int ffm_check(const rbx_field_t* fields, int F, int64_t B, FfmPack* pack, rbx_field_t* view, int* dim) {
  if (fields == nullptr) return fail(RBX_ERR_INVALID, "ffm: fields is NULL");
  if (B < 0) return fail(RBX_ERR_INVALID, "ffm: batch=%lld", static_cast<long long>(B));
  if (F < 2 || F > RBX_MAX_FIELDS) return fail(RBX_ERR_UNSUPPORTED, "ffm: n_fields=%d not in [2,%d]", F, RBX_MAX_FIELDS);
  const int D = fields[0].dim;
  if (D <= 0 || D % 4 != 0 || D > 128) return fail(RBX_ERR_UNSUPPORTED, "ffm: dim=%d is not a multiple of 4 in [4,128]", D);
  if (F * D > 1024) return fail(RBX_ERR_UNSUPPORTED, "ffm: F*D=%d exceeds the reduce's lane group (1024 floats)", F * D);
  for (int i = 0; i < F; ++i) {
    const rbx_field_t& f = fields[i];
    if (f.kind != RBX_FIELD_CATEGORICAL || f.pool != RBX_POOL_NONE || f.seq_len != 1)
      return fail(RBX_ERR_UNSUPPORTED, "ffm: field %d is not a one-id categorical feature", i);
    if (f.dim != D) return fail(RBX_ERR_UNSUPPORTED, "ffm: field %d has dim %d, field 0 has %d", i, f.dim, D);
    if (f.ids == nullptr || f.table == nullptr) return fail(RBX_ERR_INVALID, "ffm: field %d: NULL ids / table", i);
    if (f.ids_dtype < RBX_I32 || f.ids_dtype > RBX_F64) return fail(RBX_ERR_INVALID, "ffm: field %d: bad ids_dtype", i);
    if (f.table_stride != 0 && f.table_stride != D)
      return fail(RBX_ERR_UNSUPPORTED, "ffm: field %d: table_stride %lld != dim", i, static_cast<long long>(f.table_stride));
    if (f.padding_idx != RBX_NO_ID) return fail(RBX_ERR_UNSUPPORTED, "ffm: field %d has a padding_idx", i);
    if (f.vocab < F || f.vocab > INT_MAX)
      return fail(RBX_ERR_INVALID, "ffm: field %d: vocab=%lld holds no block of %d rows", i, static_cast<long long>(f.vocab), F);
    if ((reinterpret_cast<uintptr_t>(f.table) & 15) != 0 || (reinterpret_cast<uintptr_t>(f.grad) & 15) != 0)
      return fail(RBX_ERR_UNSUPPORTED, "ffm: field %d: table / grad is not 16-byte aligned", i);
    for (int k = 0; k < i; ++k)
      if (fields[k].table == f.table) return fail(RBX_ERR_UNSUPPORTED, "ffm: fields %d and %d share a table", k, i);
    FfmField& q = pack->f[i];
    q.ids = f.ids;
    q.table = f.table;
    q.stride_b = f.ids_stride_b;
    q.nblocks = static_cast<int>(f.vocab / F);
    q.dtype = f.ids_dtype;
    if (view != nullptr) {
      rbx_field_t& v = view[i];
      v = f;
      v.vocab = f.vocab / F;
      v.dim = F * D;
      v.out_off = 0;
      v.mask_id = RBX_NO_ID;
      v.ids_stride_l = 0;
      v.table_stride = 0;
    }
  }
  *dim = D;
  return RBX_OK;
}

static int ffm_plan(const rbx_field_t* fields, int F, int64_t B, FfmPack* pack, BwdPlan* p, int* dim, size_t* bytes) {
  rbx_field_t view[RBX_MAX_FIELDS];
  int rc = ffm_check(fields, F, B, pack, view, dim);
  if (rc != RBX_OK) return rc;
  rc = make_plan(view, F, B, nullptr, 0, p);
  if (rc != RBX_OK) return rc;
  if (!p->vec) return fail(RBX_ERR_UNSUPPORTED, "ffm: the gradients are not float4-addressable");
  *bytes = ffm_align(p->bytes) + sizeof(FfmPack);
  return RBX_OK;
}

template <bool REDUCE>
static void ffm_launch_fwd(const FfmPack& pack, int F, int D, int64_t B, float* out, int64_t stride, int* status,
                           hipStream_t s) {
  const int spw = 64 / F;
  const unsigned n_tasks = static_cast<unsigned>((B + spw - 1) / spw);
  unsigned blocks = (n_tasks + 3) / 4;
  if (blocks > static_cast<unsigned>(kCUs * 8)) blocks = kCUs * 8;
#define RBX_FFM_FWD(D4C)                                                                                              \
  hipLaunchKernelGGL((ffm_fwd_kernel<D4C, REDUCE>), dim3(blocks), dim3(256), 0, s, pack, F, D, static_cast<long long>(B), \
                     out, static_cast<long long>(stride), status, spw, n_tasks)
  switch (D / 4) {
    case 1: RBX_FFM_FWD(1); break;
    case 2: RBX_FFM_FWD(2); break;
    case 4: RBX_FFM_FWD(4); break;
    case 8: RBX_FFM_FWD(8); break;
    default: RBX_FFM_FWD(0); break;
  }
#undef RBX_FFM_FWD
}

}

extern "C" int rbx_ffm_fwd(const rbx_field_t* fields, int32_t n_fields, int64_t batch, int32_t reduce_sum, float* d_out,
                           int64_t out_stride_b, int32_t* d_status, void* stream) {
  using namespace rbx;
  FfmPack pack;
  int D = 0;
  int rc = ffm_check(fields, n_fields, batch, &pack, nullptr, &D);
  if (rc != RBX_OK) return rc;
  if (batch == 0) return RBX_OK;
  if (d_out == nullptr) return fail(RBX_ERR_INVALID, "ffm_fwd: d_out is NULL");
  const int64_t P = static_cast<int64_t>(n_fields) * (n_fields - 1) / 2;
  if (out_stride_b < (reduce_sum ? P : P * D)) return fail(RBX_ERR_INVALID, "ffm_fwd: out_stride_b below the row width");
  if (batch / (64 / n_fields) >= (1ll << 31)) return fail(RBX_ERR_UNSUPPORTED, "ffm_fwd: batch too large");
  if (!reduce_sum && ((reinterpret_cast<uintptr_t>(d_out) & 15) != 0 || out_stride_b % 4 != 0))
    return fail(RBX_ERR_UNSUPPORTED, "ffm_fwd: d_out must be 16-byte aligned with a row stride that is a multiple of 4");
  if (reduce_sum && (reinterpret_cast<uintptr_t>(d_out) & 3) != 0) return fail(RBX_ERR_UNSUPPORTED, "ffm_fwd: misaligned d_out");
  if (reduce_sum) ffm_launch_fwd<true>(pack, n_fields, D, batch, d_out, out_stride_b, d_status, as_stream(stream));
  else ffm_launch_fwd<false>(pack, n_fields, D, batch, d_out, out_stride_b, d_status, as_stream(stream));
  return check_launch("ffm_fwd_kernel");
}

extern "C" size_t rbx_ffm_bwd_workspace_size(const rbx_field_t* fields, int32_t n_fields, int64_t batch) {
  using namespace rbx;
  FfmPack pack;
  BwdPlan p;
  int D = 0;
  size_t bytes = 0;
  if (ffm_plan(fields, n_fields, batch, &pack, &p, &D, &bytes) != RBX_OK) return 0;
  return bytes;
}

extern "C" int rbx_ffm_sort(const rbx_field_t* fields, int32_t n_fields, int64_t batch, void* d_workspace,
                            size_t workspace_bytes, int32_t* d_status, void* stream) {
  using namespace rbx;
  FfmPack pack;
  BwdPlan p;
  int D = 0;
  size_t bytes = 0;
  int rc = ffm_plan(fields, n_fields, batch, &pack, &p, &D, &bytes);
  if (rc != RBX_OK) return rc;
  if (batch == 0 || p.n_lookups == 0) return RBX_OK;
  if (d_workspace == nullptr || workspace_bytes < bytes)
    return fail(RBX_ERR_WORKSPACE, "ffm_sort: workspace %zu B < required %zu B", workspace_bytes, bytes);
  return run_sort(p, static_cast<char*>(d_workspace), d_status, as_stream(stream));
}

extern "C" int rbx_ffm_bwd(const rbx_field_t* fields, int32_t n_fields, int64_t batch, int32_t reduce_sum,
                           const float* d_dout, int64_t dout_stride_b, int32_t accumulate, void* d_workspace,
                           size_t workspace_bytes, void* stream) {
  using namespace rbx;
  FfmPack pack;
  BwdPlan p;
  int D = 0;
  size_t bytes = 0;
  int rc = ffm_plan(fields, n_fields, batch, &pack, &p, &D, &bytes);
  if (rc != RBX_OK) return rc;
  if (batch == 0 || p.n_lookups == 0) return RBX_OK;
  if (d_dout == nullptr) return fail(RBX_ERR_INVALID, "ffm_bwd: d_dout is NULL");
  const int64_t P = static_cast<int64_t>(n_fields) * (n_fields - 1) / 2;
  if (dout_stride_b < (reduce_sum ? P : P * D)) return fail(RBX_ERR_INVALID, "ffm_bwd: dout_stride_b below the row width");
  if (!reduce_sum && ((reinterpret_cast<uintptr_t>(d_dout) & 15) != 0 || dout_stride_b % 4 != 0))
    return fail(RBX_ERR_UNSUPPORTED, "ffm_bwd: d_dout must be 16-byte aligned with a row stride that is a multiple of 4");
  if (reduce_sum && (reinterpret_cast<uintptr_t>(d_dout) & 3) != 0) return fail(RBX_ERR_UNSUPPORTED, "ffm_bwd: misaligned d_dout");
  if (d_workspace == nullptr || workspace_bytes < bytes)
    return fail(RBX_ERR_WORKSPACE, "ffm_bwd: workspace %zu B < required %zu B", workspace_bytes, bytes);
  char* ws = static_cast<char*>(d_workspace);
  hipStream_t s = as_stream(stream);
// ... 12 lines not shown
```

recbox_amd/csrc/rbx_segreduce.h:

```cpp
#pragma once
#include "rbx_bwd_common.h"

namespace rbx {

template <class F>
__device__ __forceinline__ void frag_add(F& a, const F& b) {
#pragma unroll
  for (int q = 0; q < static_cast<int>(sizeof(a.a) / sizeof(float)); ++q) a.a[q] += b.a[q];
}

constexpr unsigned kLongSlots = 512;
constexpr unsigned kLongSplit = 16;
constexpr int kFinList = 3;
#define RBX_REDUCE_WAVES 3
template <class Policy>
struct ReduceWideBatch {
  static constexpr int of(int) { return 4; }
};
template <class Policy>
struct ReduceLaneZeros {
  static constexpr bool value = false;
};
template <class Policy, int G, int NV, bool VEC>
__global__ __launch_bounds__(256, RBX_REDUCE_WAVES) void segment_reduce_kernel(const RedPack P, const int n_cat,
                                                             const typename Policy::Args args,
                                                             const unsigned* __restrict__ keys,
                                                             const unsigned* __restrict__ vals, const unsigned n,
                                                             const unsigned sentinel, float* __restrict__ head,
                                                             float* __restrict__ tail, int* __restrict__ flags,
                                                             unsigned* __restrict__ fin, const int max_dim,
                                                             const int sum_stride, const unsigned n_chunks,
                                                             const unsigned chunk) {
  __shared__ RedField sf[RBX_MAX_FIELDS];
  {
    const int words = n_cat * static_cast<int>(sizeof(RedField) / 4);
    const int* src = reinterpret_cast<const int*>(&P);
    int* dst = reinterpret_cast<int*>(sf);
    for (int i = threadIdx.x; i < words; i += blockDim.x) dst[i] = src[i];
  }
  __syncthreads();
  using F = Frag<G, NV, VEC>;
  const int lane_g = threadIdx.x % G;
  const unsigned c = blockIdx.x * (blockDim.x / G) + threadIdx.x / G;
  if (c >= n_chunks) return;
  const unsigned s = c * chunk;
  const unsigned e = (s + chunk < n) ? s + chunk : n;
  const unsigned key_before = (s > 0) ? keys[s - 1] : sentinel;
  const unsigned key_after = (e < n) ? keys[e] : sentinel;
  unsigned cur = keys[s];
  const bool open_in = (s > 0) && (cur == key_before) && (cur != sentinel);
  bool seen_boundary = false;
  unsigned cur_val = vals[s];
  F acc, pre_last;
  acc.zero();
  pre_last.zero();
  float cnt = 0.f;
  bool head_done = false;
#define RBX_REDUCE_U 8
  constexpr int U = (G * NV * F::W <= 32) ? RBX_REDUCE_U : ReduceWideBatch<Policy>::of(NV * F::W);
  for (unsigned i0 = s; i0 < e; i0 += U) {
    unsigned kk[U + 1], vv[U];
    {
      constexpr int PER = (U + G - 1) / G;
      unsigned mk[PER], mv[PER];
#pragma unroll
      for (int k = 0; k < PER; ++k) {
        const unsigned i = i0 + k * G + lane_g;
        const bool ok = (k * G + lane_g < U) && (i < e);
        mk[k] = ok ? __builtin_nontemporal_load(keys + i) : sentinel;
        mv[k] = ok ? __builtin_nontemporal_load(vals + i) : 0u;
      }
      const int gbase = (threadIdx.x & 63) & ~(G - 1);
#pragma unroll
      for (int u = 0; u < U; ++u) {
        kk[u] = __shfl(mk[u / G], gbase + (u % G), 64);
        vv[u] = __shfl(mv[u / G], gbase + (u % G), 64);
      }
    }
    kk[U] = (i0 + U < e) ? keys[i0 + U] : key_after;
    F rows[U], pre[U];
    float rc[U];
#define RBX_REDUCE_BATCHED 1
#if RBX_REDUCE_BATCHED
    float wu[U];
#pragma unroll
    for (int u = 0; u < U; ++u) {
      rows[u].zero();
      wu[u] = 0.f;
      if (kk[u] != sentinel && i0 + u < e)
        Policy::fetch(args, sf[vv[u] >> kLocalBits], vv[u] & kLocalMask, lane_g, rows[u], wu[u]);
    }
#pragma unroll
    for (int u = 0; u < U; ++u) {
      pre[u].zero();
      if (kk[u] != sentinel && i0 + u < e) {
        const unsigned nxt = (i0 + u + 1 < e) ? kk[u + 1] : key_after;
        if (nxt != kk[u]) Policy::prefetch_raw(args, sf[vv[u] >> kLocalBits], kk[u] - sf[vv[u] >> kLocalBits].row_base, lane_g, pre[u]);
      }
    }
#pragma unroll
    for (int u = 0; u < U; ++u) {
      const bool valid = kk[u] != sentinel && i0 + u < e;
      const float w = Policy::weight(args, wu[u]);
      if (valid) rows[u].scale(w); else rows[u].zero();
      rc[u] = (valid && Policy::kHasCount) ? w : 0.f;
    }
#else
#pragma unroll
    for (int u = 0; u < U; ++u) {
      rows[u].zero();
      pre[u].zero();
      rc[u] = 0.f;
      if (kk[u] != sentinel && i0 + u < e) {
        const RedField& fd = sf[vv[u] >> kLocalBits];
        Policy::contribute(args, fd, vv[u] & kLocalMask, lane_g, rows[u], rc[u]);
        const unsigned nxt = (i0 + u + 1 < e) ? kk[u + 1] : key_after;
        if (nxt != kk[u]) Policy::prefetch(args, fd, kk[u] - fd.row_base, lane_g, pre[u]);
      }
    }
#endif
#pragma unroll
    for (int u = 0; u < U; ++u) {
      if (i0 + u >= e) break;
      if (kk[u] != cur) {
        seen_boundary = true;
        acc.zero();
        cnt = 0.f;
        cur = kk[u];
        cur_val = vv[u];
      }
      frag_add(acc, rows[u]);
      cnt += rc[u];
      const unsigned nxt = (i0 + u + 1 < e) ? kk[u + 1] : key_after;
      const bool last_in_chunk = (i0 + u + 1 >= e);
      if (cur != sentinel && nxt != cur && !last_in_chunk) {
        const RedField& fd = sf[cur_val >> kLocalBits];
        if (!seen_boundary && open_in) {
          float* dst = head + static_cast<size_t>(c) * sum_stride;
          acc.store(dst, fd.dim, lane_g);
          if (Policy::kHasCount && lane_g == 0) dst[max_dim] = cnt;
          head_done = true;
        } else {
          Policy::flush(args, fd, cur - fd.row_base, acc, cnt, pre[u], lane_g);
        }
      }
      if (last_in_chunk) pre_last = pre[u];
    }
  }
  int flag = 0;
  if (cur != sentinel) {
    const RedField& fd = sf[cur_val >> kLocalBits];
    const bool open_out = (e < n) && (key_after == cur);
    const bool is_head = !seen_boundary && open_in;
    if (open_out) {
      float* dst = tail + static_cast<size_t>(c) * sum_stride;
      acc.store(dst, fd.dim, lane_g);
      if (Policy::kHasCount && lane_g == 0) dst[max_dim] = cnt;
      if (is_head) flag |= kFlagPass;
      bool zero = (cnt == 0.f);
#pragma unroll
      for (int q = 0; q < static_cast<int>(sizeof(acc.a) / sizeof(float)); ++q) zero = zero && (acc.a[q] == 0.f);
#pragma unroll
      for (int o = 1; o < G; o <<= 1) {
        if constexpr (ReduceLaneZeros<Policy>::value) {
          const int other = __shfl_xor(static_cast<int>(zero), o, 64);
          zero = zero && (other != 0);
        } else {
          zero = zero && (__shfl_xor(static_cast<int>(zero), o, 64) != 0);
        }
      }
      if (zero) flag |= kFlagZero;
    } else if (is_head) {
      float* dst = head + static_cast<size_t>(c) * sum_stride;
      acc.store(dst, fd.dim, lane_g);
      if (Policy::kHasCount && lane_g == 0) dst[max_dim] = cnt;
      flag |= kFlagFin;
    } else {
      Policy::flush(args, fd, cur - fd.row_base, acc, cnt, pre_last, lane_g);
    }
  }
  if (head_done) flag |= kFlagFin;
  if (lane_g == 0) {
    flags[c] = flag;
    if (flag & kFlagFin) fin[kFinList + atomicAdd(fin, 1u)] = c;
  }
}

constexpr int kShortHops = 8;

template <class Policy, int G, int NV, bool VEC>
__global__ __launch_bounds__(256) void segment_fixup_short_kernel(const RedPack P, const typename Policy::Args args,
                                                                  const unsigned* __restrict__ keys,
                                                                  const unsigned* __restrict__ vals,
                                                                  const float* __restrict__ head,
                                                                  const float* __restrict__ tail,
                                                                  const int* __restrict__ flags,
                                                                  unsigned* __restrict__ fin, const int max_dim,
                                                                  const int sum_stride, const unsigned n_chunks,
                                                                  const unsigned chunk) {
  using F = Frag<G, NV, VEC>;
  const int lane_g = threadIdx.x % G;
  const unsigned ngroups = gridDim.x * (blockDim.x / G);
  const unsigned count = fin[0];
  for (unsigned idx = blockIdx.x * (blockDim.x / G) + threadIdx.x / G; idx < count; idx += ngroups) {
    const unsigned c = fin[kFinList + idx];
    int hops = 0;
    bool closed = false;
    for (long long j = static_cast<long long>(c) - 1; j >= 0 && hops < kShortHops; --j) {
      ++hops;
      if (!(flags[j] & kFlagPass)) { closed = true; break; }
    }
    if (!closed && c > 0) {
      if (lane_g == 0) {
        const unsigned pos = atomicAdd(fin + 1, 1u);
        fin[kFinList + n_chunks + pos] = c;
        if (pos < kLongSlots) fin[kFinList + 2 * n_chunks + pos] = 0;
      }
      continue;
    }
    const unsigned s = c * chunk;
    const unsigned key = keys[s];
    const RedField fd = P.f[vals[s] >> kLocalBits];
    F acc, pre;
    acc.zero();
    pre.zero();
    Policy::prefetch(args, fd, key - fd.row_base, lane_g, pre);
    const float* src = head + static_cast<size_t>(c) * sum_stride;
    acc.add_from(src, fd.dim, lane_g);
    float cnt = Policy::kHasCount ? src[max_dim] : 0.f;
    for (int h = 1; h <= hops; ++h) {
      if (flags[c - h] & kFlagZero) continue;
      const float* t = tail + static_cast<size_t>(c - h) * sum_stride;
      acc.add_from(t, fd.dim, lane_g);
      if (Policy::kHasCount) cnt += t[max_dim];
    }
    Policy::flush(args, fd, key - fd.row_base, acc, cnt, pre, lane_g);
  }
}

template <class Policy, int G, int NV, bool VEC>
__global__ __launch_bounds__(256) void segment_fixup_long_kernel(const RedPack P, const typename Policy::Args args,
                                                                 const unsigned* __restrict__ keys,
                                                                 const unsigned* __restrict__ vals,
                                                                 const float* __restrict__ head,
                                                                 const float* __restrict__ tail,
                                                                 const int* __restrict__ flags,
                                                                 unsigned* __restrict__ fin, const int max_dim,
                                                                 const int sum_stride, const unsigned n_chunks,
                                                                 const unsigned chunk, float* __restrict__ lpart) {
  using F = Frag<G, NV, VEC>;
  constexpr int NGB = 256 / G;
  constexpr int R = (2 * G < 8) ? 8 : ((2 * G > 32) ? 32 : 2 * G);
  constexpr int NA = NV * F::W;
  constexpr int kNone = 1 << 30;
  __shared__ int s_stop[4];
  __shared__ float s_part[4][G * NA + 1];
  __shared__ unsigned s_last;
  const int lane = threadIdx.x & 63, wid = threadIdx.x >> 6;
  const int gi = threadIdx.x / G, lane_g = threadIdx.x % G;
  const unsigned count = fin[1];
  unsigned KW = 1;
  if (count > 0 && count <= kLongSlots && count * 2 <= gridDim.x && lpart != nullptr) {
    KW = gridDim.x / count;
    KW = KW > kLongSplit ? kLongSplit : KW;
    if (count * KW > kLongSlots) KW = 1;
  }
  unsigned* lcnt = fin + kFinList + 2 * static_cast<size_t>(n_chunks);
  const unsigned items = count * KW;
  const unsigned needed = items == 0 ? 1u : (items < gridDim.x ? items : gridDim.x);
  if (blockIdx.x >= needed) return;
  for (unsigned item = blockIdx.x; item < items; item += gridDim.x) {
    const unsigned idx = item / KW, jw = item % KW;
    const unsigned c = fin[kFinList + n_chunks + idx];
    const unsigned s = c * chunk;
    const unsigned key = keys[s];
    unsigned kw = 1;
    if (KW > 1) {
      if (threadIdx.x == 0) {
        unsigned lo = 0, hi = c;
        while (lo < hi) {
          const unsigned mid = (lo + hi) >> 1;
          if (keys[(static_cast<size_t>(mid) + 1) * chunk - 1] >= key) hi = mid;
          else lo = mid + 1;
        }
        unsigned w = ((c - lo + NGB * R - 1) / (NGB * R)) / 2;
        s_last = w < 1 ? 1u : (w > KW ? KW : w);
      }
      __syncthreads();
      kw = s_last;
      __syncthreads();
      if (jw >= kw) continue;
    }
    const RedField fd = P.f[vals[s] >> kLocalBits];
    F acc, pre;
    acc.zero();
    pre.zero();
    float cnt = 0.f;
    if (gi == 0 && jw == 0) {
      if (kw == 1) Policy::prefetch(args, fd, key - fd.row_base, lane_g, pre);
      const float* src = head + static_cast<size_t>(c) * sum_stride;
      acc.add_from(src, fd.dim, lane_g);
      if (Policy::kHasCount) cnt = src[max_dim];
    }
    long long jbase = static_cast<long long>(c) - 1 - static_cast<long long>(jw) * (NGB * R);
    bool adjoining = jw == 0;
    while (jbase >= 0) {
      if (!adjoining && keys[(static_cast<size_t>(jbase) + 1) * chunk - 1] != key) break;
      adjoining = kw == 1;
      int fl[R];
      int first_stop = kNone;
#pragma unroll
      for (int r = 0; r < R; ++r) {
        const long long j = jbase - (static_cast<long long>(gi) * R + r);
        fl[r] = (j >= 0) ? flags[j] : 0;
      }
#pragma unroll
      for (int r = R - 1; r >= 0; --r) {
        const long long j = jbase - (static_cast<long long>(gi) * R + r);
        if (j < 0 || !(fl[r] & kFlagPass)) first_stop = gi * R + r;
      }
      int wmin = first_stop;
#pragma unroll
      for (int o = 1; o < 64; o <<= 1) {
        const int other = __shfl_xor(wmin, o, 64);
        wmin = other < wmin ? other : wmin;
      }
      if (lane == 0) s_stop[wid] = wmin;
      __syncthreads();
      int t = s_stop[0];
#pragma unroll
      for (int w = 1; w < 4; ++w) t = (s_stop[w] < t) ? s_stop[w] : t;
      F part;
      part.zero();
      float pc = 0.f;
#pragma unroll
      for (int r = 0; r < R; ++r) {
        const int d = gi * R + r;
        const long long j = jbase - d;
        if (j >= 0 && d <= t && !(fl[r] & kFlagZero)) {
          const float* src = tail + static_cast<size_t>(j) * sum_stride;
          part.add_from(src, fd.dim, lane_g);
          if (Policy::kHasCount) pc += src[max_dim];
        }
      }
#pragma unroll
      for (int o = G; o < 64; o <<= 1) {
#pragma unroll
        for (int q = 0; q < NA; ++q) part.a[q] += __shfl_xor(part.a[q], o, 64);
        pc += __shfl_xor(pc, o, 64);
      }
      if (lane < G) {
#pragma unroll
        for (int q = 0; q < NA; ++q) s_part[wid][lane * NA + q] = part.a[q];
        if (lane == 0) s_part[wid][G * NA] = pc;
      }
      __syncthreads();
      if (gi == 0) {
#pragma unroll
        for (int w = 0; w < 4; ++w) {
#pragma unroll
          for (int q = 0; q < NA; ++q) acc.a[q] += s_part[w][lane_g * NA + q];
          cnt += s_part[w][G * NA];
        }
      }
      __syncthreads();
      if (t != kNone) break;
      jbase -= static_cast<long long>(kw) * (NGB * R);
    }
    if (kw == 1) {
      if (gi == 0) Policy::flush(args, fd, key - fd.row_base, acc, cnt, pre, lane_g);
      continue;
    }
    if (gi == 0) {
      float* slot = lpart + static_cast<size_t>(item) * sum_stride;
      acc.store(slot, fd.dim, lane_g);
      if (Policy::kHasCount && lane_g == 0) slot[max_dim] = cnt;
    }
    __threadfence();
    __syncthreads();
    if (threadIdx.x == 0) s_last = (atomicAdd(lcnt + idx, 1u) == kw - 1) ? 1u : 0u;
    __syncthreads();
    if (s_last) {
      __threadfence();
      if (gi == 0) {
        F tot;
        tot.zero();
        float tc = 0.f;
        Policy::prefetch(args, fd, key - fd.row_base, lane_g, pre);
        for (unsigned w = 0; w < kw; ++w) {
          const float* slot = lpart + (static_cast<size_t>(idx) * KW + w) * sum_stride;
          tot.add_from(slot, fd.dim, lane_g);
          if (Policy::kHasCount) tc += slot[max_dim];
        }
        Policy::flush(args, fd, key - fd.row_base, tot, tc, pre, lane_g);
      }
    }
    __syncthreads();
  }
  __syncthreads();
  if (threadIdx.x == 0) {
    if (atomicAdd(fin + 2, 1u) == needed - 1) {
      fin[0] = 0;
      fin[1] = 0;
      fin[2] = 0;
    }
  }
}

template <class Policy, int G, int NV, bool VEC>
static int launch_reduce(const BwdPlan& p, const typename Policy::Args& args, const unsigned* keys,
                         const unsigned* vals, char* ws, hipStream_t s) {
  const int groups_per_block = 256 / G;
  const unsigned blocks = (p.n_chunks + groups_per_block - 1) / groups_per_block;
  float* head = reinterpret_cast<float*>(ws + p.off_head);
  float* tail = reinterpret_cast<float*>(ws + p.off_tail);
  int* flags = reinterpret_cast<int*>(ws + p.off_flags);
  unsigned* fin = reinterpret_cast<unsigned*>(ws + p.off_fin);
  hipLaunchKernelGGL((segment_reduce_kernel<Policy, G, NV, VEC>), dim3(blocks), dim3(256), 0, s, p.red, p.n_cat, args,
                     keys, vals, p.n_lookups, p.total_rows, head, tail, flags, fin, p.max_dim, p.sum_stride,
                     p.n_chunks, static_cast<unsigned>(p.chunk));
  int rc = check_launch("segment_reduce_kernel");
  if (rc != RBX_OK) return rc;
  unsigned short_blocks = blocks;
  if (short_blocks > static_cast<unsigned>(kCUs * 8)) short_blocks = kCUs * 8;
  hipLaunchKernelGGL((segment_fixup_short_kernel<Policy, G, NV, VEC>), dim3(short_blocks), dim3(256), 0, s, p.red, args,
                     keys, vals, head, tail, flags, fin, p.max_dim, p.sum_stride, p.n_chunks,
                     static_cast<unsigned>(p.chunk));
  unsigned long_blocks = p.n_chunks;
  if (long_blocks > p.long_cap) long_blocks = p.long_cap;
  hipLaunchKernelGGL((segment_fixup_long_kernel<Policy, G, NV, VEC>), dim3(long_blocks), dim3(256), 0, s, p.red, args,
                     keys, vals, head, tail, flags, fin, p.max_dim, p.sum_stride, p.n_chunks,
                     static_cast<unsigned>(p.chunk), reinterpret_cast<float*>(ws + p.off_long));
  return check_launch("segment_fixup kernels");
}

template <class Policy, bool VEC>
static int dispatch_reduce(const BwdPlan& p, const typename Policy::Args& args, const unsigned* keys,
                           const unsigned* vals, char* ws, hipStream_t s) {
  const int units = VEC ? p.max_dim / 4 : p.max_dim;
  switch (pow2_ceil(units)) {
    case 1: return launch_reduce<Policy, 1, 1, VEC>(p, args, keys, vals, ws, s);
    case 2: return launch_reduce<Policy, 2, 1, VEC>(p, args, keys, vals, ws, s);
    case 4: return launch_reduce<Policy, 4, 1, VEC>(p, args, keys, vals, ws, s);
    case 8: return launch_reduce<Policy, 8, 1, VEC>(p, args, keys, vals, ws, s);
    case 16: return launch_reduce<Policy, 16, 1, VEC>(p, args, keys, vals, ws, s);
    case 32: return launch_reduce<Policy, 32, 1, VEC>(p, args, keys, vals, ws, s);
    case 64: return launch_reduce<Policy, 64, 1, VEC>(p, args, keys, vals, ws, s);
    case 128: return launch_reduce<Policy, 64, 2, VEC>(p, args, keys, vals, ws, s);
    case 256: return launch_reduce<Policy, 64, 4, VEC>(p, args, keys, vals, ws, s);
    default: return fail(RBX_ERR_UNSUPPORTED, "embedding dim too large for one lane group");
  }
}

template <bool VEC>
__device__ __forceinline__ void rezero_rows_block(const RedField* sf, const unsigned block, const unsigned* __restrict__ keys,
                                                  const unsigned* __restrict__ vals, const unsigned n,
                                                  const unsigned sentinel, const int lanes) {
  typedef float v4f __attribute__((ext_vector_type(4)));
  constexpr int W = VEC ? 4 : 1;
  const unsigned i = block * blockDim.x + threadIdx.x;
  float* row_ptr = nullptr;
  int dim = 0;
  if (i < n) {
    const unsigned key = keys[i];
    const unsigned prev = (i > 0) ? keys[i - 1] : sentinel;
    const unsigned val = vals[i];
    if (key < sentinel && key != prev) {
      const RedField& fd = sf[val >> kLocalBits];
      const size_t row = key - fd.row_base;
      if (fd.grad != nullptr) {
        row_ptr = fd.grad + row * fd.dim;
        dim = fd.dim;
      }
      if (fd.grad2 != nullptr) fd.grad2[row] = 0.f;
    }
  }
  const int lane = threadIdx.x & 63;
  const int lane_g = lane % lanes, group = lane / lanes, per_step = 64 / lanes;
  for (int base = 0; base < 64; base += per_step) {
    const int src = base + group;
    float* dst = reinterpret_cast<float*>(__shfl(reinterpret_cast<unsigned long long>(row_ptr), src, 64));
    const int d = __shfl(dim, src, 64);
    for (int e = lane_g * W; e < d; e += lanes * W) {
      if constexpr (VEC) {
        const v4f z = {0.f, 0.f, 0.f, 0.f};
        __builtin_nontemporal_store(z, reinterpret_cast<v4f*>(dst + e));
      } else {
        dst[e] = 0.f;
      }
    }
  }
}

template <bool VEC>
__global__ __launch_bounds__(256) void rezero_rows_kernel(const RedPack P, const int n_cat, const unsigned* __restrict__ keys,
                                                        const unsigned* __restrict__ vals, const unsigned n,
                                                        const unsigned sentinel, const int lanes) {
  __shared__ RedField sf[RBX_MAX_FIELDS];
  {
    const int words = n_cat * static_cast<int>(sizeof(RedField) / 4);
    const int* src = reinterpret_cast<const int*>(&P);
    int* dst = reinterpret_cast<int*>(sf);
    for (int i = threadIdx.x; i < words; i += blockDim.x) dst[i] = src[i];
  }
  __syncthreads();
  rezero_rows_block<VEC>(sf, blockIdx.x, keys, vals, n, sentinel, lanes);
}


static inline int rezero_lanes(const BwdPlan& p) {
  const int width = p.vec ? (p.max_dim + 3) / 4 : p.max_dim;
  int lanes = 1;
  while (lanes < width && lanes < 64) lanes *= 2;
  return lanes;
}

static inline int launch_rezero(const BwdPlan& p, const char* ws, hipStream_t s) {
  const int cur = p.passes & 1;
  const unsigned* keys = reinterpret_cast<const unsigned*>(ws + p.off_keys[cur]);
  const unsigned* vals = reinterpret_cast<const unsigned*>(ws + p.off_vals[cur]);
  const int lanes = rezero_lanes(p);
  const unsigned blocks = (p.n_lookups + 255) / 256;
  if (p.vec)
    hipLaunchKernelGGL(rezero_rows_kernel<true>, dim3(blocks), dim3(256), 0, s, p.red, p.n_cat, keys, vals, p.n_lookups,
                       p.total_rows, lanes);
  else
    hipLaunchKernelGGL(rezero_rows_kernel<false>, dim3(blocks), dim3(256), 0, s, p.red, p.n_cat, keys, vals, p.n_lookups,
                       p.total_rows, lanes);
  return check_launch("rezero_rows_kernel");
}

}
```

recbox_amd/ops.py:

```python
import ctypes
import os
import weakref

import torch

from . import _lib
from ._lib import (FIELD_CATEGORICAL, FIELD_DENSE, FIELD_NUMERIC, POOL_CONCAT, POOL_MAX, POOL_MEAN_ID, POOL_MEAN_VALUE,
                   POOL_NONE, POOL_SUM, POOL_SUM_ID, RBX_NO_ID, check, lib)

_DTYPE_CODE = {torch.int32: _lib.RBX_I32, torch.int64: _lib.RBX_I64,
               torch.float32: _lib.RBX_F32, torch.float64: _lib.RBX_F64}


class config(object):
    sort_before_forward = os.environ.get("RECBOX_AMD_SORT_FIRST", "1") != "0"
    dw_beside_lookup = os.environ.get("RECBOX_AMD_DW_BESIDE", "1") != "0"
    db_before_dx = True
    check_ids = os.environ.get("RECBOX_AMD_CHECK_IDS", "1") != "0"
    fork_in_capture = True
    share_sorts = True
    defer_id_check = os.environ.get("RECBOX_AMD_DEFER_IDS", "1") != "0"
    fuse_sigmoid_bce = os.environ.get("RECBOX_AMD_FUSE_SIGMOID_BCE", "1") != "0"
    fuse_sublayers = os.environ.get("RECBOX_AMD_FUSE_SUBLAYERS", "1") != "0"
    seqblock_chains = os.environ.get("RECBOX_AMD_SEQBLOCK", "1") != "0"
# ... 192 lines not shown
        st = torch.cuda.Stream(device=device)
        _side_streams[key] = st
    return st


class _SortMemo(object):
    __slots__ = ("a", "b", "n", "fm", "ws", "B", "ids", "stream", "serial", "captured")


_sort_memo = {}
_sort_serial = [0]
sort_counts = {"sorted": 0, "shared": 0}


def _enqueue_sort(desc, keep, B, ws, nbytes, st, sort_call):
    if not config.share_sorts:
        return sort_call()
    dev = keep[0].device.index
    memo = _sort_memo.get(dev)
    _sort_serial[0] += 1
    capturing = torch.cuda.is_current_stream_capturing()
    fresh = (memo is not None and memo.captured and memo.serial == _sort_serial[0] - 1) if capturing else True
    if (memo is not None and fresh and memo.B == B and memo.ws is not ws and memo.stream == st.value
            and all(t._version == v for t, v in memo.ids)):
        rc = lib.rbx_sort_share(memo.a, memo.b, memo.n, memo.fm, _ptr(memo.ws), desc[0], desc[1], desc[2], desc[3],
                                _ptr(ws), nbytes, B, st)
        if rc != _lib.RBX_ERR_UNSUPPORTED:
            sort_counts["shared"] += 1
            return rc
    sort_counts["sorted"] += 1
    rc = sort_call()
    if rc == _lib.RBX_OK:
        memo = _SortMemo()
        memo.a = type(desc[0]).from_buffer_copy(desc[0]) if desc[0] is not None else None
        memo.b = type(desc[1]).from_buffer_copy(desc[1]) if desc[1] is not None else None
        memo.n, memo.fm, memo.ws, memo.B, memo.stream = desc[2], desc[3], ws, B, st.value
        memo.ids = [(t, t._version) for t in keep]
        memo.serial, memo.captured = _sort_serial[0], capturing
        _sort_memo[dev] = memo
    return rc


class TouchedRows(object):
    __slots__ = ("kind", "plans", "inputs", "params", "grads", "ws", "ws_bytes", "B", "serial", "tables", "pool")


touched = {}
_touched_serial = [0]


def _note_touched(kind, plans, inputs, params, grads, ws, ws_bytes, B, tables=None, pool=None):
    rec = TouchedRows()
    grads = tuple([g.detach() if g is not None else None for g in group] for group in grads)
    rec.kind, rec.plans, rec.inputs, rec.params, rec.grads = kind, plans, list(inputs), params, grads
    rec.ws, rec.ws_bytes, rec.B, rec.tables, rec.pool = ws, int(ws_bytes), int(B), tables, pool
    _touched_serial[0] += 1
    rec.serial = _touched_serial[0]
    for group in params:
        for p in group:
            touched[id(p)] = rec


touched_ids = {}
_ids_pass = [0, False, None]


def _ids_pass_over():
    _ids_pass[0] += 1
    _ids_pass[1] = False


def _note_ids(plan, inputs, params, grads, want, ids_of=None):
    now = _pass_id()
    if _ids_pass[1] and now >= 0 and _ids_pass[2] != now:
        _ids_pass_over()
    if not _ids_pass[1]:
        _ids_pass[1], _ids_pass[2] = True, now
        torch.autograd.Variable._execution_engine.queue_callback(_ids_pass_over)
    for k, (p, g, w) in enumerate(zip(params, grads, want)):
        if not w or g is None:
            continue
        ids = ids_of(k) if ids_of is not None else \
            [t for sp, t in zip(plan.specs, inputs) if sp.kind == _lib.FIELD_CATEGORICAL and sp.param == k]
        ent = touched_ids.get(id(p))
        if ent is not None and ent[0] == g.data_ptr() and ent[2] == _ids_pass[0]:
            ent[1].extend(ids)
        else:
            touched_ids[id(p)] = (g.data_ptr(), ids, _ids_pass[0])


def _forget_sort(ws):
    for dev, memo in list(_sort_memo.items()):
        if memo.ws is ws:
            del _sort_memo[dev]


class _EarlySort(object):

    def __init__(self, device, ws_bytes, launch, ws=None, first=None):
        cur = torch.cuda.current_stream(device)
        self.ws = ws if ws is not None else torch.empty(max(int(ws_bytes), 1), dtype=torch.uint8, device=device)
        self.ws_bytes = int(ws_bytes)
        self.event = None
        self.event_first = None
        self.side = None
        if torch.cuda.is_current_stream_capturing() and not config.fork_in_capture:
            st = ctypes.c_void_p(cur.cuda_stream)
            if first is not None:
                check(first(self.ws, st))
            check(launch(self.ws, st))
            return
        side = _side_stream(device)
        side.wait_stream(cur)
        st = ctypes.c_void_p(side.cuda_stream)
        if first is not None:
            check(first(self.ws, st))
            self.event_first = side.record_event()
        check(launch(self.ws, st))
        self.event = side.record_event()
        self.side = side
        self.ws.record_stream(side)

    def join(self):
        if self.event is not None:
            torch.cuda.current_stream().wait_event(self.event)


_deferred_status = {}


def _status_word(device):
    if config.check_ids:
        return torch.zeros(1, dtype=torch.int32, device=device)
    if not config.defer_id_check:
        return None
    key = device.index if device.index is not None else torch.cuda.current_device()
    t = _deferred_status.get(key)
    if t is None:
        t = _deferred_status[key] = torch.zeros(1, dtype=torch.int32, device=device)
    return t


def _check_status(status):
    if status is not None and config.check_ids and int(status.item()) != 0:
        raise IndexError("index out of range in self")


def fm_quad_kernel(enable=None):
    return bool(lib.rbx_fm_quad(-1 if enable is None else int(bool(enable))))


def sort_chained(enable=None):
    return bool(lib.rbx_sort_chained(-1 if enable is None else int(bool(enable))))


_bag_long = [1024]


def bag_long_threshold(value=None):
    old = _bag_long[0]
    if value is not None:
        value = int(value)
        if value < 0:
            raise ValueError("bag_long_threshold must be >= 0, got %d" % value)
        _bag_long[0] = value
    return old


def check_deferred_ids():
    bad = False
    for t in _deferred_status.values():
        if int(t.item()) != 0:
            bad = True
            t.zero_()
    if bad:
        raise IndexError("index out of range in self (reported late: recbox_amd.ops.config.check_ids was off)")


class _EmbedLookup(torch.autograd.Function):

    @staticmethod
    def forward(ctx, plan, n_inputs, train, pad_rows, *tensors):
        inputs, params = tensors[:n_inputs], tensors[n_inputs:]
        for p in params:
            _require_cuda(p, "embedding parameter")
            if p.dtype != torch.float32 or not p.is_contiguous():
                raise RuntimeError("recbox_amd: embedding parameters must be contiguous fp32")
        B, keep = plan.bind_inputs(inputs)
        plan.bind_params(params)
        dev = params[0].device if params else keep[0].device
        out = _padded_rows(B, plan.width, dev) if pad_rows else torch.empty((B, plan.width), dtype=torch.float32, device=dev)
        row_scale = torch.empty((plan.n, B), dtype=torch.float32, device=dev) if plan.needs_row_scale else None
        status = _status_word(dev)
        check(_timed(("embed_fwd", plan.n, plan.width, B),
                     lambda: lib.rbx_embed_fwd(plan.arr, plan.n, B, _ptr(out), out.stride(0) if B > 1 else plan.width,
                                               _ptr(row_scale), _ptr(status), _stream())))
        _check_status(status)
        ctx.plan, ctx.inputs, ctx.row_scale, ctx.B = plan, keep, row_scale, B
        ctx.params = params
        ctx.sort = None
        if train:
            _note_readers(ctx, params)
        if B > 0 and train:
            placeholders = [p if p.requires_grad else None for p in params]
            plan.bind_params(params, placeholders)
            ws_bytes = lib.rbx_embed_bwd_workspace_size(plan.arr, plan.n, B)
            pool = _GradPool.claim(_EmbedLookup._pool_for(plan, params, dev)
                                   if config.reuse_grad_buffers == "all" else None)

            def sort(ws, nbytes, st):
                return _enqueue_sort((plan.arr, None, plan.n, 0), keep, B, ws, nbytes, st,
                                     lambda: lib.rbx_embed_sort(plan.arr, plan.n, B, _ptr(ws), nbytes, None, st))

            if ws_bytes > 0 and pool is None:
                ctx.sort = _EarlySort(dev, ws_bytes, lambda ws, st: sort(ws, ws_bytes, st))
            elif ws_bytes > 0:
                def rezero(st):
                    plan.bind_params(params, pool.bind_views(list(params)))
                    rc = lib.rbx_embed_rezero(plan.arr, plan.n, pool.dirty_batch, _ptr(pool.ws), pool.ws_bytes, st)
                    pool.dirty_batch = 0
                    plan.bind_params(params, placeholders)
                    return rc

                pool.early_sort(ctx, dev, ws_bytes, rezero, sort)
        return out

    @staticmethod
    def _pool_for(plan, params, dev):
        params = list(params)
        pool = getattr(plan, "_grad_pool", None)
        if pool is None or not pool.matches(params):
            by_id = set(sp.param for sp in plan.specs if sp.kind == FIELD_CATEGORICAL)
            pool = plan._grad_pool = _GradPool(params, [i in by_id for i in range(len(params))], dev)
        return pool

    @staticmethod
    def backward(ctx, dout):
        plan, params, B = ctx.plan, ctx.params, ctx.B
        if dout.stride(1) != 1 or dout.dtype != torch.float32:
            dout = dout.contiguous().float()
        need = [i + 4 + len(ctx.inputs) for i in range(len(params))]
        want = [ctx.needs_input_grad[j] for j in need]
        want_now = [p.requires_grad for p in params]
        pool, grads = None, None
        adopted = _adopt_grads(ctx, params, want) if B > 0 else None
        if adopted is not None:
            grads = adopted
        elif getattr(ctx, "pool", None) is not None:
            pool, grads = ctx.pool.backward_grads(ctx, params, want, want_now == list(want) and B > 0)
        if grads is None:
            grads = _flat_zero_grads(params, want, dout.device)
        if B == 0:
            return (None, None, None, None) + (None,) * len(ctx.inputs) + tuple(grads)
        plan.bind_inputs(ctx.inputs)
        plan.bind_params(params, grads)
        if ctx.sort is not None and want_now == list(want):
            ctx.sort.join()
            ws, ws_bytes = ctx.sort.ws, ctx.sort.ws_bytes
        else:
            ws_bytes = lib.rbx_embed_bwd_workspace_size(plan.arr, plan.n, B)
            ws = torch.empty(max(ws_bytes, 1), dtype=torch.uint8, device=dout.device)
            check(lib.rbx_embed_sort(plan.arr, plan.n, B, _ptr(ws), ws_bytes, None, _stream()))
        check(lib.rbx_embed_bwd(plan.arr, plan.n, B, _ptr(dout), dout.stride(0) if B > 1 else plan.width,
                                _ptr(ctx.row_scale), 1 if adopted is not None else 0, _ptr(ws), ws_bytes, _stream()))
        if pool is not None:
            pool.done(B)
        _forget_sort(ws)
        if config.track_touched_rows:
            _note_ids(plan, ctx.inputs, params, grads, want)
        if adopted is not None:
            for p, w in zip(params, want):
                if w:
                    touched.pop(id(p), None)
            return (None, None, None, None) + (None,) * len(ctx.inputs) + (None,) * len(params)
        if config.track_touched_rows:
            _note_touched("embed", (plan,), ctx.inputs, (list(params),), (list(grads),), ws, ws_bytes, B)
        _publish_grads(ctx, params, grads)
        return (None, None, None, None) + (None,) * len(ctx.inputs) + tuple(grads)


def embed_lookup(plan, inputs, params, pad_rows=False):
    train = torch.is_grad_enabled() and any(p.requires_grad for p in params)
    return _EmbedLookup.apply(plan, len(inputs), train, pad_rows, *inputs, *params)


class Bags(object):
    __slots__ = ("indices", "offsets", "weights")

    def __init__(self, indices, offsets, weights=None):
        _require_cuda(indices, "bag indices")
        _require_cuda(offsets, "bag offsets")
        if weights is not None:
            _require_cuda(weights, "bag weights")
            if weights.dtype != torch.float32:
                raise TypeError("bag weights must be float32, got %s" % weights.dtype)
            if weights.dim() != 1 or weights.numel() != indices.numel() or weights.device != indices.device:
                raise ValueError("bag weights must be 1-D with one entry per index on the indices' device, got %s on %s for "
                                 "%d indices on %s" % (tuple(weights.shape), weights.device, indices.numel(), indices.device))
            weights = weights.contiguous()
        if indices.device != offsets.device:
            raise ValueError("bag indices and offsets live on different devices (%s, %s)" % (indices.device, offsets.device))
        if indices.dim() != 1 or offsets.dim() != 1:
            raise ValueError("bag indices and offsets must be 1-D, got %s and %s" % (tuple(indices.shape), tuple(offsets.shape)))
        if offsets.numel() < 1:
            raise ValueError("bag offsets need B + 1 >= 1 entries")
        if indices.dtype not in _DTYPE_CODE:
# ... 3752 lines not shown
```

Before: 325.9 million samples/s.

## Replace head/tail segment fixup with run-ownership reduce and direct long-run scan

The segmented gradient reduce no longer writes per-chunk head/tail partials and flags for a separate short-fixup kernel. Instead, the chunk that starts a run owns it and reads past its chunk end, up to kShortHops chunks, to finish short runs directly. Longer runs are handed to the long-fixup kernel, which now scans the sorted keys directly instead of summing stored tails. This drops one kernel launch and the head/tail/flag workspace traffic, in exchange for redundant key reads past chunk boundaries and a changed long-run path.

New measurement: 324.7 million samples/s. Within noise of the previous version (-0.4%).

```diff
diff --git a/include/recbox_hip.h b/include/recbox_hip.h
--- a/include/recbox_hip.h
+++ b/include/recbox_hip.h
@@ -65,6 +65,8 @@
                   int32_t* d_status, void* stream);
 
 size_t rbx_embed_bwd_workspace_size(const rbx_field_t* fields, int32_t n_fields, int64_t batch);
+int32_t rbx_reduce_chunk(int64_t n_lookups);
+int32_t rbx_reduce_short_hops(void);
 int rbx_embed_sort(const rbx_field_t* fields, int32_t n_fields, int64_t batch,
                    void* d_workspace, size_t workspace_bytes, int32_t* d_status, void* stream);
 int rbx_embed_bwd(const rbx_field_t* fields, int32_t n_fields, int64_t batch,
diff --git a/recbox_amd/_lib.py b/recbox_amd/_lib.py
--- a/recbox_amd/_lib.py
+++ b/recbox_amd/_lib.py
@@ -96,6 +96,8 @@
     "rbx_version": (ctypes.c_int, []),
     "rbx_embed_fwd": (ctypes.c_int, [_FP, _i32, _i64, _P, _i64, _P, _P, _P]),
     "rbx_embed_bwd_workspace_size": (_sz, [_FP, _i32, _i64]),
+    "rbx_reduce_chunk": (_i32, [_i64]),
+    "rbx_reduce_short_hops": (_i32, []),
     "rbx_embed_sort": (ctypes.c_int, [_FP, _i32, _i64, _P, _sz, _P, _P]),
     "rbx_embed_bwd": (ctypes.c_int, [_FP, _i32, _i64, _P, _i64, _P, _i32, _P, _sz, _P]),
     "rbx_embed_bwd_indexed": (ctypes.c_int, [_FP, _i32, _i64, _P, _i64, _P, _P, _i32, _P, _sz, _P]),
diff --git a/recbox_amd/csrc/rbx_bwd_common.h b/recbox_amd/csrc/rbx_bwd_common.h
--- a/recbox_amd/csrc/rbx_bwd_common.h
+++ b/recbox_amd/csrc/rbx_bwd_common.h
@@ -14,6 +14,10 @@
 constexpr int kMaxRadixBits = RBX_MAX_RADIX_BITS;
 #define RBX_CHUNK 40
 constexpr int kChunk = RBX_CHUNK;
+static inline int reduce_chunk_of(unsigned long long n_lookups) {
+  int c = static_cast<int>(n_lookups / 32768u) / 8 * 8;
+  return c < 16 ? 16 : (c > kChunk ? kChunk : c);
+}
 constexpr unsigned kLocalBits = 26;
 constexpr unsigned kLocalMask = (1u << kLocalBits) - 1u;
 constexpr int kNumSamples = 256;
@@ -98,7 +102,7 @@
   SegPack segs;
   int max_dim = 1;
   bool vec = true;
-  size_t off_keys[2], off_vals[2], off_hist, off_ssum, off_head, off_tail, off_flags, off_fin, off_long, off_num, bytes;
+  size_t off_keys[2], off_vals[2], off_hist, off_ssum, off_fin, off_long, off_num, bytes;
   bool chained = false;
   unsigned n_tiles = 0, n_chunks = 0, num_blocks = 0;
   unsigned long_cap = kCUs * 2;
@@ -231,9 +235,4 @@
   }
 };
 
-constexpr int kFlagFin = 1;
-constexpr int kFlagPass = 2;
-constexpr int kFlagZero = 4;
-
-
-}
+}
diff --git a/recbox_amd/csrc/rbx_embed_bwd.hip b/recbox_amd/csrc/rbx_embed_bwd.hip
--- a/recbox_amd/csrc/rbx_embed_bwd.hip
+++ b/recbox_amd/csrc/rbx_embed_bwd.hip
@@ -150,12 +150,7 @@
       S.first_pass[g] = static_cast<unsigned char>(p->passes - need);
     }
   }
-  {
-    int c = static_cast<int>(p->n_lookups / 32768u) / 8 * 8;
-    if (c < 16) c = 16;
-    if (c > kChunk) c = kChunk;
-    p->chunk = c;
-  }
+  p->chunk = reduce_chunk_of(p->n_lookups);
   p->n_chunks = (p->n_lookups + p->chunk - 1) / p->chunk;
   p->num_blocks = static_cast<unsigned>((B + kNumSamples - 1) / kNumSamples);
   size_t o = 0;
@@ -172,10 +167,7 @@
                   : align_up(static_cast<size_t>(p->n_tiles) * radix * 4 + 4, 256);
   p->off_ssum = o; o += align_up((static_cast<size_t>(p->n_tiles) * radix / 4096 + 2) * 4, 256);
   p->sum_stride = p->max_dim + extra_dim;
-  p->off_head = o; o += align_up(static_cast<size_t>(p->n_chunks) * p->sum_stride * 4, 256);
-  p->off_tail = o; o += align_up(static_cast<size_t>(p->n_chunks) * p->sum_stride * 4, 256);
-  p->off_flags = o; o += align_up(static_cast<size_t>(p->n_chunks) * 4, 256);
-  p->off_fin = o; o += align_up((2 * static_cast<size_t>(p->n_chunks) + 3 + kLongSlots) * 4, 256);
+  p->off_fin = o; o += align_up((kFinList + kLongSlots + long_list_cap(p->n_chunks)) * 4, 256);
   p->off_long = o; o += align_up(static_cast<size_t>(kLongSlots) * p->sum_stride * 4, 256);
   p->off_num = o; o += align_up(static_cast<size_t>(p->n_num) * p->num_blocks * p->max_dim * 4, 256);
   p->bytes = o + 256;
@@ -719,6 +711,12 @@
   return was;
 }
 
+extern "C" int32_t rbx_reduce_chunk(int64_t n_lookups) {
+  return n_lookups < 0 ? 0 : rbx::reduce_chunk_of(static_cast<unsigned long long>(n_lookups));
+}
+
+extern "C" int32_t rbx_reduce_short_hops(void) { return rbx::kShortHops; }
+
 extern "C" size_t rbx_embed_bwd_workspace_size(const rbx_field_t* fields, int32_t n_fields, int64_t batch) {
   rbx::BwdPlan p;
   if (rbx::make_plan(fields, n_fields, batch, nullptr, 0, &p) != RBX_OK) return 0;
diff --git a/recbox_amd/csrc/rbx_embed_csr.hip b/recbox_amd/csrc/rbx_embed_csr.hip
--- a/recbox_amd/csrc/rbx_embed_csr.hip
+++ b/recbox_amd/csrc/rbx_embed_csr.hip
@@ -850,10 +850,6 @@
 struct ReduceWideBatch<MaxBagPolicy> {
   static constexpr int of(int per_lane) { return per_lane > 8 ? 2 : 4; }
 };
-template <>
-struct ReduceLaneZeros<MaxBagPolicy> {
-  static constexpr bool value = true;
-};
 
 static int csr_sort(const rbx_bag_t* bags, int n_bags, int64_t batch, void* d_workspace, size_t workspace_bytes,
                     int* d_status, hipStream_t s, bool pos) {
diff --git a/recbox_amd/csrc/rbx_ffm.hip b/recbox_amd/csrc/rbx_ffm.hip
--- a/recbox_amd/csrc/rbx_ffm.hip
+++ b/recbox_amd/csrc/rbx_ffm.hip
@@ -162,10 +162,6 @@
 struct ReduceWideBatch<FfmPolicy> {
   static constexpr int of(int per_lane) { return per_lane >= 16 ? 2 : 4; }
 };
-template <>
-struct ReduceLaneZeros<FfmPolicy> {
-  static constexpr bool value = true;
-};
 
 __global__ __launch_bounds__(64) void ffm_pack_kernel(const FfmPack P, const int F, FfmField* __restrict__ dst) {
   const int words = F * static_cast<int>(sizeof(FfmField) / 4);
diff --git a/recbox_amd/csrc/rbx_segreduce.h b/recbox_amd/csrc/rbx_segreduce.h
--- a/recbox_amd/csrc/rbx_segreduce.h
+++ b/recbox_amd/csrc/rbx_segreduce.h
@@ -11,26 +11,28 @@
 
 constexpr unsigned kLongSlots = 512;
 constexpr unsigned kLongSplit = 16;
+constexpr int kLongBlock = 32;
 constexpr int kFinList = 3;
+constexpr int kShortHops = 8;
+static inline size_t long_list_cap(unsigned n_chunks) { return n_chunks / kShortHops + 2; }
 #define RBX_REDUCE_WAVES 3
 template <class Policy>
 struct ReduceWideBatch {
   static constexpr int of(int) { return 4; }
 };
-template <class Policy>
-struct ReduceLaneZeros {
-  static constexpr bool value = false;
-};
+#define RBX_REDUCE_U 8
+template <class Policy, int G, int NV, bool VEC>
+constexpr int reduce_batch() {
+  return (G * NV * (VEC ? 4 : 1) <= 32) ? RBX_REDUCE_U : ReduceWideBatch<Policy>::of(NV * (VEC ? 4 : 1));
+}
+
 template <class Policy, int G, int NV, bool VEC>
 __global__ __launch_bounds__(256, RBX_REDUCE_WAVES) void segment_reduce_kernel(const RedPack P, const int n_cat,
                                                              const typename Policy::Args args,
                                                              const unsigned* __restrict__ keys,
                                                              const unsigned* __restrict__ vals, const unsigned n,
-                                                             const unsigned sentinel, float* __restrict__ head,
-                                                             float* __restrict__ tail, int* __restrict__ flags,
-                                                             unsigned* __restrict__ fin, const int max_dim,
-                                                             const int sum_stride, const unsigned n_chunks,
-                                                             const unsigned chunk) {
+                                                             const unsigned sentinel, unsigned* __restrict__ fin,
+                                                             const unsigned n_chunks, const unsigned chunk) {
   __shared__ RedField sf[RBX_MAX_FIELDS];
   {
     const int words = n_cat * static_cast<int>(sizeof(RedField) / 4);
@@ -46,19 +48,18 @@
   const unsigned s = c * chunk;
   const unsigned e = (s + chunk < n) ? s + chunk : n;
   const unsigned key_before = (s > 0) ? keys[s - 1] : sentinel;
+  const unsigned key_last = keys[e - 1];
   const unsigned key_after = (e < n) ? keys[e] : sentinel;
-  unsigned cur = keys[s];
-  const bool open_in = (s > 0) && (cur == key_before) && (cur != sentinel);
-  bool seen_boundary = false;
-  unsigned cur_val = vals[s];
-  F acc, pre_last;
+  const bool follow = key_after == key_last && key_last != sentinel && key_last != key_before;
+  const unsigned lim = (e + static_cast<unsigned>(kShortHops) * chunk < n) ? e + static_cast<unsigned>(kShortHops) * chunk : n;
+  unsigned hi = e;
+  unsigned cur = sentinel, cur_val = 0, run_start = 0;
+  F acc;
   acc.zero();
-  pre_last.zero();
   float cnt = 0.f;
-  bool head_done = false;
-#define RBX_REDUCE_U 8
-  constexpr int U = (G * NV * F::W <= 32) ? RBX_REDUCE_U : ReduceWideBatch<Policy>::of(NV * F::W);
-  for (unsigned i0 = s; i0 < e; i0 += U) {
+  constexpr int U = reduce_batch<Policy, G, NV, VEC>();
+  unsigned i0 = s;
+  while (true) {
     unsigned kk[U + 1], vv[U];
     {
       constexpr int PER = (U + G - 1) / G;
@@ -66,7 +67,7 @@
 #pragma unroll
       for (int k = 0; k < PER; ++k) {
         const unsigned i = i0 + k * G + lane_g;
-        const bool ok = (k * G + lane_g < U) && (i < e);
+        const bool ok = (k * G + lane_g < U) && (i < hi);
         mk[k] = ok ? __builtin_nontemporal_load(keys + i) : sentinel;
         mv[k] = ok ? __builtin_nontemporal_load(vals + i) : 0u;
       }
@@ -77,296 +78,198 @@
         vv[u] = __shfl(mv[u / G], gbase + (u % G), 64);
       }
     }
-    kk[U] = (i0 + U < e) ? keys[i0 + U] : key_after;
+    const unsigned nb = i0 + U;
+    kk[U] = (nb < hi) ? keys[nb] : (hi == e ? key_after : (hi < n ? keys[hi] : sentinel));
+    bool use[U];
+#pragma unroll
+    for (int u = 0; u < U; ++u)
+      use[u] = (i0 + u < hi) && kk[u] != sentinel && kk[u] != key_before && (hi == e || kk[u] == key_last);
     F rows[U], pre[U];
     float rc[U];
-#define RBX_REDUCE_BATCHED 1
-#if RBX_REDUCE_BATCHED
     float wu[U];
 #pragma unroll
     for (int u = 0; u < U; ++u) {
       rows[u].zero();
       wu[u] = 0.f;
-      if (kk[u] != sentinel && i0 + u < e)
-        Policy::fetch(args, sf[vv[u] >> kLocalBits], vv[u] & kLocalMask, lane_g, rows[u], wu[u]);
+      if (use[u]) Policy::fetch(args, sf[vv[u] >> kLocalBits], vv[u] & kLocalMask, lane_g, rows[u], wu[u]);
     }
 #pragma unroll
     for (int u = 0; u < U; ++u) {
       pre[u].zero();
-      if (kk[u] != sentinel && i0 + u < e) {
-        const unsigned nxt = (i0 + u + 1 < e) ? kk[u + 1] : key_after;
-        if (nxt != kk[u]) Policy::prefetch_raw(args, sf[vv[u] >> kLocalBits], kk[u] - sf[vv[u] >> kLocalBits].row_base, lane_g, pre[u]);
-      }
+      const unsigned nxt = (i0 + u + 1 < hi) ? kk[u + 1] : kk[U];
+      if (use[u] && nxt != kk[u])
+        Policy::prefetch_raw(args, sf[vv[u] >> kLocalBits], kk[u] - sf[vv[u] >> kLocalBits].row_base, lane_g, pre[u]);
     }
 #pragma unroll
     for (int u = 0; u < U; ++u) {
-      const bool valid = kk[u] != sentinel && i0 + u < e;
       const float w = Policy::weight(args, wu[u]);
-      if (valid) rows[u].scale(w); else rows[u].zero();
-      rc[u] = (valid && Policy::kHasCount) ? w : 0.f;
-    }
-#else
+      if (use[u]) rows[u].scale(w); else rows[u].zero();
+      rc[u] = (use[u] && Policy::kHasCount) ? w : 0.f;
+    }
+    bool handed = false;
 #pragma unroll
     for (int u = 0; u < U; ++u) {
-      rows[u].zero();
-      pre[u].zero();
-      rc[u] = 0.f;
-      if (kk[u] != sentinel && i0 + u < e) {
-        const RedField& fd = sf[vv[u] >> kLocalBits];
-        Policy::contribute(args, fd, vv[u] & kLocalMask, lane_g, rows[u], rc[u]);
-        const unsigned nxt = (i0 + u + 1 < e) ? kk[u + 1] : key_after;
-        if (nxt != kk[u]) Policy::prefetch(args, fd, kk[u] - fd.row_base, lane_g, pre[u]);
-      }
-    }
-#endif
-#pragma unroll
-    for (int u = 0; u < U; ++u) {
-      if (i0 + u >= e) break;
+      if (!use[u]) continue;
       if (kk[u] != cur) {
-        seen_boundary = true;
         acc.zero();
         cnt = 0.f;
         cur = kk[u];
         cur_val = vv[u];
+        run_start = i0 + u;
       }
       frag_add(acc, rows[u]);
       cnt += rc[u];
-      const unsigned nxt = (i0 + u + 1 < e) ? kk[u + 1] : key_after;
-      const bool last_in_chunk = (i0 + u + 1 >= e);
-      if (cur != sentinel && nxt != cur && !last_in_chunk) {
+      const unsigned nxt = (i0 + u + 1 < hi) ? kk[u + 1] : kk[U];
+      if (nxt != cur) {
         const RedField& fd = sf[cur_val >> kLocalBits];
-        if (!seen_boundary && open_in) {
-          float* dst = head + static_cast<size_t>(c) * sum_stride;
-          acc.store(dst, fd.dim, lane_g);
-          if (Policy::kHasCount && lane_g == 0) dst[max_dim] = cnt;
-          head_done = true;
-        } else {
-          Policy::flush(args, fd, cur - fd.row_base, acc, cnt, pre[u], lane_g);
+        Policy::flush(args, fd, cur - fd.row_base, acc, cnt, pre[u], lane_g);
+      } else if (i0 + u + 1 == lim) {
+        if (lane_g == 0) {
+          const unsigned pos = atomicAdd(fin + 1, 1u);
+          fin[kFinList + kLongSlots + pos] = run_start;
+          if (pos < kLongSlots) fin[kFinList + pos] = 0;
         }
-      }
-      if (last_in_chunk) pre_last = pre[u];
-    }
-  }
-  int flag = 0;
-  if (cur != sentinel) {
-    const RedField& fd = sf[cur_val >> kLocalBits];
-    const bool open_out = (e < n) && (key_after == cur);
-    const bool is_head = !seen_boundary && open_in;
-    if (open_out) {
-      float* dst = tail + static_cast<size_t>(c) * sum_stride;
-      acc.store(dst, fd.dim, lane_g);
-      if (Policy::kHasCount && lane_g == 0) dst[max_dim] = cnt;
-      if (is_head) flag |= kFlagPass;
-      bool zero = (cnt == 0.f);
-#pragma unroll
-      for (int q = 0; q < static_cast<int>(sizeof(acc.a) / sizeof(float)); ++q) zero = zero && (acc.a[q] == 0.f);
-#pragma unroll
-      for (int o = 1; o < G; o <<= 1) {
-        if constexpr (ReduceLaneZeros<Policy>::value) {
-          const int other = __shfl_xor(static_cast<int>(zero), o, 64);
-          zero = zero && (other != 0);
-        } else {
-          zero = zero && (__shfl_xor(static_cast<int>(zero), o, 64) != 0);
-        }
-      }
-      if (zero) flag |= kFlagZero;
-    } else if (is_head) {
-      float* dst = head + static_cast<size_t>(c) * sum_stride;
-      acc.store(dst, fd.dim, lane_g);
-      if (Policy::kHasCount && lane_g == 0) dst[max_dim] = cnt;
-      flag |= kFlagFin;
-    } else {
-      Policy::flush(args, fd, cur - fd.row_base, acc, cnt, pre_last, lane_g);
-    }
-  }
-  if (head_done) flag |= kFlagFin;
-  if (lane_g == 0) {
-    flags[c] = flag;
-    if (flag & kFlagFin) fin[kFinList + atomicAdd(fin, 1u)] = c;
-  }
-}
-
-constexpr int kShortHops = 8;
+        handed = true;
+      }
+    }
+    if (handed) break;
+    i0 = (nb < hi) ? nb : hi;
+    if (i0 == hi) {
+      if (hi != e || !follow || lim == e) break;
+      hi = lim;
+    } else if (hi != e && kk[U] != key_last) {
+      break;
+    }
+  }
+}
 
 template <class Policy, int G, int NV, bool VEC>
-__global__ __launch_bounds__(256) void segment_fixup_short_kernel(const RedPack P, const typename Policy::Args args,
-                                                                  const unsigned* __restrict__ keys,
-                                                                  const unsigned* __restrict__ vals,
-                                                                  const float* __restrict__ head,
-                                                                  const float* __restrict__ tail,
-                                                                  const int* __restrict__ flags,
-                                                                  unsigned* __restrict__ fin, const int max_dim,
-                                                                  const int sum_stride, const unsigned n_chunks,
-                                                                  const unsigned chunk) {
-  using F = Frag<G, NV, VEC>;
-  const int lane_g = threadIdx.x % G;
-  const unsigned ngroups = gridDim.x * (blockDim.x / G);
-  const unsigned count = fin[0];
-  for (unsigned idx = blockIdx.x * (blockDim.x / G) + threadIdx.x / G; idx < count; idx += ngroups) {
-    const unsigned c = fin[kFinList + idx];
-    int hops = 0;
-    bool closed = false;
-    for (long long j = static_cast<long long>(c) - 1; j >= 0 && hops < kShortHops; --j) {
-      ++hops;
-      if (!(flags[j] & kFlagPass)) { closed = true; break; }
-    }
-    if (!closed && c > 0) {
-      if (lane_g == 0) {
-        const unsigned pos = atomicAdd(fin + 1, 1u);
-        fin[kFinList + n_chunks + pos] = c;
-        if (pos < kLongSlots) fin[kFinList + 2 * n_chunks + pos] = 0;
-      }
-      continue;
-    }
-    const unsigned s = c * chunk;
-    const unsigned key = keys[s];
-    const RedField fd = P.f[vals[s] >> kLocalBits];
-    F acc, pre;
-    acc.zero();
-    pre.zero();
-    Policy::prefetch(args, fd, key - fd.row_base, lane_g, pre);
-    const float* src = head + static_cast<size_t>(c) * sum_stride;
-    acc.add_from(src, fd.dim, lane_g);
-    float cnt = Policy::kHasCount ? src[max_dim] : 0.f;
-    for (int h = 1; h <= hops; ++h) {
-      if (flags[c - h] & kFlagZero) continue;
-      const float* t = tail + static_cast<size_t>(c - h) * sum_stride;
-      acc.add_from(t, fd.dim, lane_g);
-      if (Policy::kHasCount) cnt += t[max_dim];
-    }
-    Policy::flush(args, fd, key - fd.row_base, acc, cnt, pre, lane_g);
-  }
-}
-
-template <class Policy, int G, int NV, bool VEC>
-__global__ __launch_bounds__(256) void segment_fixup_long_kernel(const RedPack P, const typename Policy::Args args,
+__global__ __launch_bounds__(256) void segment_fixup_long_kernel(const RedPack P, const int n_cat,
+                                                                 const typename Policy::Args args,
                                                                  const unsigned* __restrict__ keys,
-                                                                 const unsigned* __restrict__ vals,
-                                                                 const float* __restrict__ head,
-                                                                 const float* __restrict__ tail,
-                                                                 const int* __restrict__ flags,
+                                                                 const unsigned* __restrict__ vals, const unsigned n,
                                                                  unsigned* __restrict__ fin, const int max_dim,
-                                                                 const int sum_stride, const unsigned n_chunks,
-                                                                 const unsigned chunk, float* __restrict__ lpart) {
+                                                                 const int sum_stride, float* __restrict__ lpart) {
   using F = Frag<G, NV, VEC>;
   constexpr int NGB = 256 / G;
-  constexpr int R = (2 * G < 8) ? 8 : ((2 * G > 32) ? 32 : 2 * G);
+  constexpr int U = reduce_batch<Policy, G, NV, VEC>();
+  constexpr unsigned WIN = NGB * U;
   constexpr int NA = NV * F::W;
-  constexpr int kNone = 1 << 30;
-  __shared__ int s_stop[4];
   __shared__ float s_part[4][G * NA + 1];
   __shared__ unsigned s_last;
+  __shared__ RedField sf[RBX_MAX_FIELDS];
+  {
+    const int words = n_cat * static_cast<int>(sizeof(RedField) / 4);
+    const int* src = reinterpret_cast<const int*>(&P);
+    int* dst = reinterpret_cast<int*>(sf);
+    for (int i = threadIdx.x; i < words; i += blockDim.x) dst[i] = src[i];
+  }
+  __syncthreads();
   const int lane = threadIdx.x & 63, wid = threadIdx.x >> 6;
   const int gi = threadIdx.x / G, lane_g = threadIdx.x % G;
-  const unsigned count = fin[1];
+  const unsigned count = __atomic_load_n(fin + 1, __ATOMIC_RELAXED);
   unsigned KW = 1;
   if (count > 0 && count <= kLongSlots && count * 2 <= gridDim.x && lpart != nullptr) {
     KW = gridDim.x / count;
     KW = KW > kLongSplit ? kLongSplit : KW;
     if (count * KW > kLongSlots) KW = 1;
   }
-  unsigned* lcnt = fin + kFinList + 2 * static_cast<size_t>(n_chunks);
+  unsigned* lcnt = fin + kFinList;
+  const unsigned* list = fin + kFinList + kLongSlots;
   const unsigned items = count * KW;
   const unsigned needed = items == 0 ? 1u : (items < gridDim.x ? items : gridDim.x);
   if (blockIdx.x >= needed) return;
   for (unsigned item = blockIdx.x; item < items; item += gridDim.x) {
     const unsigned idx = item / KW, jw = item % KW;
-    const unsigned c = fin[kFinList + n_chunks + idx];
-    const unsigned s = c * chunk;
-    const unsigned key = keys[s];
+    const unsigned start = list[idx];
+    const unsigned key = keys[start];
     unsigned kw = 1;
     if (KW > 1) {
-      if (threadIdx.x == 0) {
-        unsigned lo = 0, hi = c;
-        while (lo < hi) {
-          const unsigned mid = (lo + hi) >> 1;
-          if (keys[(static_cast<size_t>(mid) + 1) * chunk - 1] >= key) hi = mid;
-          else lo = mid + 1;
-        }
-        unsigned w = ((c - lo + NGB * R - 1) / (NGB * R)) / 2;
-        s_last = w < 1 ? 1u : (w > KW ? KW : w);
+      if (wid == 0) {
+        const unsigned long long pos = static_cast<unsigned long long>(start) + 2ull * lane * WIN;
+        const bool in = lane >= 1 && lane < static_cast<int>(KW) && pos < n && keys[pos] == key;
+        const unsigned long long m = __ballot(in);
+        if (lane == 0) s_last = 1u + static_cast<unsigned>(__popcll(m));
       }
       __syncthreads();
       kw = s_last;
       __syncthreads();
       if (jw >= kw) continue;
     }
-    const RedField fd = P.f[vals[s] >> kLocalBits];
+    const RedField& fd = sf[vals[start] >> kLocalBits];
     F acc, pre;
     acc.zero();
     pre.zero();
     float cnt = 0.f;
-    if (gi == 0 && jw == 0) {
-      if (kw == 1) Policy::prefetch(args, fd, key - fd.row_base, lane_g, pre);
-      const float* src = head + static_cast<size_t>(c) * sum_stride;
-      acc.add_from(src, fd.dim, lane_g);
-      if (Policy::kHasCount) cnt = src[max_dim];
-    }
-    long long jbase = static_cast<long long>(c) - 1 - static_cast<long long>(jw) * (NGB * R);
-    bool adjoining = jw == 0;
-    while (jbase >= 0) {
-      if (!adjoining && keys[(static_cast<size_t>(jbase) + 1) * chunk - 1] != key) break;
-      adjoining = kw == 1;
-      int fl[R];
-      int first_stop = kNone;
-#pragma unroll
-      for (int r = 0; r < R; ++r) {
-        const long long j = jbase - (static_cast<long long>(gi) * R + r);
-        fl[r] = (j >= 0) ? flags[j] : 0;
-      }
-#pragma unroll
-      for (int r = R - 1; r >= 0; --r) {
-        const long long j = jbase - (static_cast<long long>(gi) * R + r);
-        if (j < 0 || !(fl[r] & kFlagPass)) first_stop = gi * R + r;
-      }
-      int wmin = first_stop;
-#pragma unroll
-      for (int o = 1; o < 64; o <<= 1) {
-        const int other = __shfl_xor(wmin, o, 64);
-        wmin = other < wmin ? other : wmin;
-      }
-      if (lane == 0) s_stop[wid] = wmin;
-      __syncthreads();
-      int t = s_stop[0];
-#pragma unroll
-      for (int w = 1; w < 4; ++w) t = (s_stop[w] < t) ? s_stop[w] : t;
-      F part;
-      part.zero();
-      float pc = 0.f;
-#pragma unroll
-      for (int r = 0; r < R; ++r) {
-        const int d = gi * R + r;
-        const long long j = jbase - d;
-        if (j >= 0 && d <= t && !(fl[r] & kFlagZero)) {
-          const float* src = tail + static_cast<size_t>(j) * sum_stride;
-          part.add_from(src, fd.dim, lane_g);
-          if (Policy::kHasCount) pc += src[max_dim];
-        }
-      }
-#pragma unroll
-      for (int o = G; o < 64; o <<= 1) {
-#pragma unroll
-        for (int q = 0; q < NA; ++q) part.a[q] += __shfl_xor(part.a[q], o, 64);
-        pc += __shfl_xor(pc, o, 64);
-      }
-      if (lane < G) {
-#pragma unroll
-        for (int q = 0; q < NA; ++q) s_part[wid][lane * NA + q] = part.a[q];
-        if (lane == 0) s_part[wid][G * NA] = pc;
-      }
-      __syncthreads();
-      if (gi == 0) {
-#pragma unroll
-        for (int w = 0; w < 4; ++w) {
-#pragma unroll
-          for (int q = 0; q < NA; ++q) acc.a[q] += s_part[w][lane_g * NA + q];
-          cnt += s_part[w][G * NA];
-        }
-      }
-      __syncthreads();
-      if (t != kNone) break;
-      jbase -= static_cast<long long>(kw) * (NGB * R);
-    }
+    if (gi == 0 && kw == 1) Policy::prefetch(args, fd, key - fd.row_base, lane_g, pre);
+    F blk;
+    blk.zero();
+    float blk_cnt = 0.f;
+    int in_blk = 0;
+    for (unsigned long long pos = static_cast<unsigned long long>(start) + (static_cast<unsigned long long>(jw) * NGB + gi) * U;
+         pos < n; pos += static_cast<unsigned long long>(kw) * WIN) {
+      unsigned kk[U], vv[U];
+#pragma unroll
+      for (int u = 0; u < U; ++u) {
+        const bool ok = pos + u < n;
+        kk[u] = ok ? keys[pos + u] : ~key;
+        vv[u] = ok ? vals[pos + u] : 0u;
+      }
+      if (kk[0] != key) break;
+      F rows[U];
+      float wu[U];
+#pragma unroll
+      for (int u = 0; u < U; ++u) {
+        rows[u].zero();
+        wu[u] = 0.f;
+        if (kk[u] == key) Policy::fetch(args, sf[vv[u] >> kLocalBits], vv[u] & kLocalMask, lane_g, rows[u], wu[u]);
+      }
+      F bs;
+      bs.zero();
+      float bc = 0.f;
+#pragma unroll
+      for (int u = 0; u < U; ++u) {
+        if (kk[u] != key) continue;
+        const float w = Policy::weight(args, wu[u]);
+        rows[u].scale(w);
+        frag_add(bs, rows[u]);
+        if (Policy::kHasCount) bc += w;
+      }
+      frag_add(blk, bs);
+      blk_cnt += bc;
+      if (++in_blk == kLongBlock) {
+        frag_add(acc, blk);
+        cnt += blk_cnt;
+        blk.zero();
+        blk_cnt = 0.f;
+        in_blk = 0;
+      }
+    }
+    frag_add(acc, blk);
+    cnt += blk_cnt;
+#pragma unroll
+    for (int o = G; o < 64; o <<= 1) {
+#pragma unroll
+      for (int q = 0; q < NA; ++q) acc.a[q] += __shfl_xor(acc.a[q], o, 64);
+      cnt += __shfl_xor(cnt, o, 64);
+    }
+    if (lane < G) {
+#pragma unroll
+      for (int q = 0; q < NA; ++q) s_part[wid][lane * NA + q] = acc.a[q];
+      if (lane == 0) s_part[wid][G * NA] = cnt;
+    }
+    __syncthreads();
+    if (gi == 0) {
+      acc.zero();
+      cnt = 0.f;
+#pragma unroll
+      for (int w = 0; w < 4; ++w) {
+#pragma unroll
+        for (int q = 0; q < NA; ++q) acc.a[q] += s_part[w][lane_g * NA + q];
+        cnt += s_part[w][G * NA];
+      }
+    }
+    __syncthreads();
     if (kw == 1) {
       if (gi == 0) Policy::flush(args, fd, key - fd.row_base, acc, cnt, pre, lane_g);
       continue;
@@ -380,7 +283,9 @@
     __syncthreads();
     if (threadIdx.x == 0) s_last = (atomicAdd(lcnt + idx, 1u) == kw - 1) ? 1u : 0u;
     __syncthreads();
-    if (s_last) {
+    const bool last = s_last != 0;
+    __syncthreads();
+    if (last) {
       __threadfence();
       if (gi == 0) {
         F tot;
@@ -395,7 +300,6 @@
         Policy::flush(args, fd, key - fd.row_base, tot, tc, pre, lane_g);
       }
     }
-    __syncthreads();
   }
   __syncthreads();
   if (threadIdx.x == 0) {
@@ -412,26 +316,16 @@
                          const unsigned* vals, char* ws, hipStream_t s) {
   const int groups_per_block = 256 / G;
   const unsigned blocks = (p.n_chunks + groups_per_block - 1) / groups_per_block;
-  float* head = reinterpret_cast<float*>(ws + p.off_head);
-  float* tail = reinterpret_cast<float*>(ws + p.off_tail);
-  int* flags = reinterpret_cast<int*>(ws + p.off_flags);
   unsigned* fin = reinterpret_cast<unsigned*>(ws + p.off_fin);
   hipLaunchKernelGGL((segment_reduce_kernel<Policy, G, NV, VEC>), dim3(blocks), dim3(256), 0, s, p.red, p.n_cat, args,
-                     keys, vals, p.n_lookups, p.total_rows, head, tail, flags, fin, p.max_dim, p.sum_stride,
-                     p.n_chunks, static_cast<unsigned>(p.chunk));
+                     keys, vals, p.n_lookups, p.total_rows, fin, p.n_chunks, static_cast<unsigned>(p.chunk));
   int rc = check_launch("segment_reduce_kernel");
   if (rc != RBX_OK) return rc;
-  unsigned short_blocks = blocks;
-  if (short_blocks > static_cast<unsigned>(kCUs * 8)) short_blocks = kCUs * 8;
-  hipLaunchKernelGGL((segment_fixup_short_kernel<Policy, G, NV, VEC>), dim3(short_blocks), dim3(256), 0, s, p.red, args,
-                     keys, vals, head, tail, flags, fin, p.max_dim, p.sum_stride, p.n_chunks,
-                     static_cast<unsigned>(p.chunk));
   unsigned long_blocks = p.n_chunks;
   if (long_blocks > p.long_cap) long_blocks = p.long_cap;
-  hipLaunchKernelGGL((segment_fixup_long_kernel<Policy, G, NV, VEC>), dim3(long_blocks), dim3(256), 0, s, p.red, args,
-                     keys, vals, head, tail, flags, fin, p.max_dim, p.sum_stride, p.n_chunks,
-                     static_cast<unsigned>(p.chunk), reinterpret_cast<float*>(ws + p.off_long));
-  return check_launch("segment_fixup kernels");
+  hipLaunchKernelGGL((segment_fixup_long_kernel<Policy, G, NV, VEC>), dim3(long_blocks), dim3(256), 0, s, p.red, p.n_cat,
+                     args, keys, vals, p.n_lookups, fin, p.max_dim, p.sum_stride, reinterpret_cast<float*>(ws + p.off_long));
+  return check_launch("segment_fixup_long_kernel");
 }
 
 template <class Policy, bool VEC>
diff --git a/recbox_amd/ops.py b/recbox_amd/ops.py
--- a/recbox_amd/ops.py
+++ b/recbox_amd/ops.py
@@ -368,6 +368,10 @@
 
 def sort_chained(enable=None):
     return bool(lib.rbx_sort_chained(-1 if enable is None else int(bool(enable))))
+
+
+def reduce_shape(n_lookups):
+    return int(lib.rbx_reduce_chunk(int(n_lookups))), int(lib.rbx_reduce_short_hops())
 
 
 _bag_long = [1024]
```
